# cgisky1980/Qwen3-TTS-Rust

Measured on AMD Instinct MI355X. Metric: audio_sec_per_s, higher is better.
Workload: dtype bf16

## Files before the change

### qwen3-tts-rust_amd/csrc/q3_bgemm.hip

```cpp
#include "q3_kernels.h"

typedef __bf16 bf16x8 __attribute__((ext_vector_type(8)));
typedef uint32_t u32x4 __attribute__((ext_vector_type(4)));

__device__ __forceinline__ float bg_wave_sum(float v) {
#pragma unroll
    for (int m = 32; m >= 1; m >>= 1) v = v + __shfl_xor(v, m);
    return v;
}

__device__ __forceinline__ size_t bg_yoff(const Q3BGemm& g, int row) {
    return g.seg_rows ? (size_t)(row / g.seg_rows) * g.seg_stride + (size_t)(row % g.seg_rows) * g.ldy : (size_t)row * g.ldy;
}
__device__ __forceinline__ float bg_gelu_erf(float x) { return 0.5f * x * (1.0f + erff(x * 0.70710678118654752f)); }

__device__ __forceinline__ u32x4 bg_ldw(const u32x4* p, bool nt) { return nt ? __builtin_nontemporal_load(p) : *p; }

__device__ __forceinline__ bf16x8 bg_q8_frag(uint32_t lo, uint32_t hi) {
    union { u32x4 u; bf16x8 v; } r;
#define Q8F(w_, b_) __float_as_uint((float)(int)(signed char)((w_) >> (8 * (b_))))
    r.u.x = (Q8F(lo, 0) >> 16) | (Q8F(lo, 1) & 0xffff0000u); r.u.y = (Q8F(lo, 2) >> 16) | (Q8F(lo, 3) & 0xffff0000u);
    r.u.z = (Q8F(hi, 0) >> 16) | (Q8F(hi, 1) & 0xffff0000u); r.u.w = (Q8F(hi, 2) >> 16) | (Q8F(hi, 3) & 0xffff0000u);
#undef Q8F
    return r.v;
}
__device__ __forceinline__ float bg_f16(uint32_t bits) { return (float)__builtin_bit_cast(_Float16, (unsigned short)bits); }

#define BG_PH(RT_, NT_) ((8 * (RT_) * (NT_) > 64 && ((RT_) * (NT_)) % 2 == 0) ? 2 : 1)
template <int RT, int NT, int D, bool NTW, bool Q8>
__global__ __launch_bounds__(512) void k_bgemm(Q3BGemm g) {
    extern __shared__ float part[];
    __shared__ float srow[64];
    Q3_STAMP(g, 0);
    constexpr int TR = RT * NT * 4;
    const int wave = threadIdx.x >> 6, lane = threadIdx.x & 63, kq = lane >> 4, r = lane & 15;
    int cg = blockIdx.x, rc = blockIdx.y;
    if (gridDim.y > 1 && (gridDim.x & 7) == 0) {
        const int id = blockIdx.x + gridDim.x * blockIdx.y, G = gridDim.y;
        rc = (id >> 3) % G; cg = (id & 7) + (id / (8 * G)) * 8;
    }
    const int nb0 = cg * NT, row0 = rc * RT * 16, kblocks = g.K >> 5, per = g.K >> 8, kb0 = wave * per;
    const int B = g.B;
    const u32x4* ap[RT];
#pragma unroll
    for (int i = 0; i < RT; ++i) {
        const int R = g.a_row0 + min(row0 + 16 * i + r, B - 1);
        ap[i] = (const u32x4*)g.a + ((size_t)(R >> 4) * kblocks + kb0) * 64 + kq * 16 + (R & 15);
    }
    const u32x4* wp[NT];
#pragma unroll
    for (int j = 0; j < NT; ++j) wp[j] = (const u32x4*)g.w + ((size_t)(nb0 + j) * kblocks + kb0) * 64 + lane;
    constexpr int NR = 2 * RT;
    float sp0[NR], sp1[NR];
    if (g.ssp) {
#pragma unroll
        for (int i = 0; i < NR; ++i) {
            const float* sp = g.ssp + (size_t)min(row0 + wave + 8 * i, B - 1) * g.ld_ssp;
            sp0[i] = lane < g.ntiles ? sp[lane] : 0.0f;
            sp1[i] = lane + 64 < g.ntiles ? sp[lane + 64] : 0.0f;
        }
    }
    constexpr int DQ = (D + 1) & ~1, DP = DQ / 2;
    u32x4 aq[Q8 ? DQ : D][RT], bq[Q8 ? DP : D][NT];
    uint32_t sc8[Q8 ? DP : 1][NT];
    const u32x4* wq[NT]; const uint32_t* sq[NT];
    const int npair = per >> 1;
    if constexpr (Q8) {
#pragma unroll
        for (int j = 0; j < NT; ++j) {
            wq[j] = (const u32x4*)g.w + ((size_t)(nb0 + j) * (kblocks >> 1) + (kb0 >> 1)) * 64 + lane;
            sq[j] = (const uint32_t*)(g.wscale + (size_t)((nb0 + j) * 16 + r) * kblocks + kb0);
        }
#pragma unroll
        for (int p = 0; p < DP; ++p) {
            const int pc = min(p, npair - 1);
#pragma unroll
            for (int j = 0; j < NT; ++j) { bq[p][j] = bg_ldw(wq[j] + (size_t)pc * 64, NTW); sc8[p][j] = sq[j][pc]; }
        }
#pragma unroll
        for (int s = 0; s < DQ; ++s) {
            const size_t so = (size_t)min(s, per - 1) * 64;
#pragma unroll
            for (int i = 0; i < RT; ++i) aq[s][i] = ap[i][so];
        }
    } else {
#pragma unroll
        for (int s = 0; s < D; ++s) {
            const size_t so = (size_t)min(s, per - 1) * 64;
#pragma unroll
            for (int j = 0; j < NT; ++j) bq[s][j] = bg_ldw(wp[j] + so, NTW);
        }
#pragma unroll
        for (int s = 0; s < D; ++s) {
            const size_t so = (size_t)min(s, per - 1) * 64;
#pragma unroll
            for (int i = 0; i < RT; ++i) aq[s][i] = ap[i][so];
        }
    }
    constexpr int NOUT = (TR * 64 + 511) / 512;
    float yres[NOUT], nwv[NOUT], bsv[NOUT], csv[NOUT];
#pragma unroll
    for (int it = 0; it < NOUT; ++it) { yres[it] = 0.0f; nwv[it] = 0.0f; bsv[it] = 0.0f; csv[it] = 1.0f; }
    if (g.epi == Q3_EPI_RESID) {
#pragma unroll
        for (int it = 0; it < NOUT; ++it) {
            const int o = threadIdx.x + it * 512;
            const int l = o & 63, e = (o >> 6) & 3, t = o >> 8, i = t / NT, j = t - i * NT;
            const int row = row0 + 16 * i + 4 * (l >> 4) + e, col = (nb0 + min(j, NT - 1)) * 16 + (l & 15);
            const bool in = o < TR * 64;
            yres[it] = (in && row < B) ? g.y[bg_yoff(g, row) + col] : 0.0f;
            if (g.nw_next) nwv[it] = in ? g.nw_next[col] : 0.0f;
            if (g.col_scale) csv[it] = in ? g.col_scale[col] : 1.0f;
        }
    }
    if (g.bias && g.epi != Q3_EPI_SWIGLU) {
#pragma unroll
        for (int it = 0; it < NOUT; ++it) {
            const int o = threadIdx.x + it * 512;
            const int l = o & 63, t = o >> 8, i = t / NT, j = t - i * NT;
            const int col = (nb0 + min(j, NT - 1)) * 16 + (l & 15);
            bsv[it] = o < TR * 64 ? g.bias[col % g.bias_n] : 0.0f;
        }
    }
    __builtin_amdgcn_sched_barrier(0);
    Q3_STAMP(g, 1);
    if (g.ssp) {
        float av[NR];
#pragma unroll
        for (int i = 0; i < NR; ++i) {
            float a = sp0[i];
            if (lane + 64 < g.ntiles) a = a + sp1[i];
            if (g.ntiles > 128) {
                const float* sp = g.ssp + (size_t)min(row0 + wave + 8 * i, B - 1) * g.ld_ssp;
                for (int t = lane + 128; t < g.ntiles; t += 64) a = a + sp[t];
            }
            av[i] = a;
        }
#pragma unroll
        for (int m = 32; m >= 1; m >>= 1)
#pragma unroll
            for (int i = 0; i < NR; ++i) av[i] = av[i] + __shfl_xor(av[i], m);
        if (lane == 0) {
#pragma unroll
            for (int i = 0; i < NR; ++i) srow[wave + 8 * i] = 1.0f / sqrtf(av[i] / (float)g.d_norm + g.eps);
        }
    }
    __builtin_amdgcn_sched_barrier(0);
    f32x4 acc[RT][NT];
#pragma unroll
    for (int i = 0; i < RT; ++i)
#pragma unroll
        for (int j = 0; j < NT; ++j) acc[i][j] = (f32x4){0.f, 0.f, 0.f, 0.f};
    if constexpr (Q8) {
        const f32x4 zero4 = (f32x4){0.f, 0.f, 0.f, 0.f};
        for (int p0 = 0; p0 < npair; p0 += DP) {
#pragma unroll
            for (int dp = 0; dp < DP; ++dp) {
                const int p = p0 + dp;
                if (p < npair) {
#pragma unroll
                    for (int h = 0; h < 2; ++h) {
                        float dsc[NT]; bf16x8 bf[NT];
#pragma unroll
                        for (int j = 0; j < NT; ++j) {
                            dsc[j] = bg_f16(h ? sc8[dp][j] >> 16 : sc8[dp][j] & 0xffffu);
                            bf[j] = h ? bg_q8_frag(bq[dp][j].z, bq[dp][j].w) : bg_q8_frag(bq[dp][j].x, bq[dp][j].y);
                        }
#pragma unroll
                        for (int i = 0; i < RT; ++i) {
                            union { u32x4 u; bf16x8 v; } a; a.u = aq[2 * dp + h][i];
#pragma unroll
                            for (int j = 0; j < NT; ++j) {
                                const f32x4 P = __builtin_amdgcn_mfma_f32_16x16x32_bf16(a.v, bf[j], zero4, 0, 0, 0);
                                acc[i][j][0] = fmaf(dsc[j], P[0], acc[i][j][0]); acc[i][j][1] = fmaf(dsc[j], P[1], acc[i][j][1]);
                                acc[i][j][2] = fmaf(dsc[j], P[2], acc[i][j][2]); acc[i][j][3] = fmaf(dsc[j], P[3], acc[i][j][3]);
                            }
                        }
                    }
                    __builtin_amdgcn_sched_barrier(0);
                    if (p + DP < npair) {
#pragma unroll
                        for (int j = 0; j < NT; ++j) { bq[dp][j] = bg_ldw(wq[j] + (size_t)(p + DP) * 64, NTW); sc8[dp][j] = sq[j][p + DP]; }
#pragma unroll
                        for (int h = 0; h < 2; ++h)
#pragma unroll
                            for (int i = 0; i < RT; ++i) aq[2 * dp + h][i] = ap[i][(size_t)(2 * (p + DP) + h) * 64];
                    }
                    __builtin_amdgcn_sched_barrier(0);
                }
            }
        }
    } else
    for (int s0 = 0; s0 < per; s0 += D) {
#pragma unroll
        for (int d = 0; d < D; ++d) {
            const int s = s0 + d;
            if (s < per) {
#pragma unroll
                for (int i = 0; i < RT; ++i) {
                    union { u32x4 u; bf16x8 v; } a; a.u = aq[d][i];
#pragma unroll
                    for (int j = 0; j < NT; ++j) {
                        union { u32x4 u; bf16x8 v; } b; b.u = bq[d][j];
                        acc[i][j] = __builtin_amdgcn_mfma_f32_16x16x32_bf16(a.v, b.v, acc[i][j], 0, 0, 0);
                    }
                }
                __builtin_amdgcn_sched_barrier(0);
#ifdef Q3_STAMPS
                if (s == 0) { asm volatile("" :: "v"(acc[0][0][0])); Q3_STAMP(g, 2); }
#endif
                if (s + D < per) {
#pragma unroll
                    for (int j = 0; j < NT; ++j) bq[d][j] = bg_ldw(wp[j] + (size_t)(s + D) * 64, NTW);
#pragma unroll
                    for (int i = 0; i < RT; ++i) aq[d][i] = ap[i][(size_t)(s + D) * 64];
                }
                __builtin_amdgcn_sched_barrier(0);
            }
        }
    }
#ifdef Q3_STAMPS
    asm volatile("" :: "v"(acc[0][0][0])); Q3_STAMP(g, 3);
#endif
    constexpr int PH = BG_PH(RT, NT), TP = RT * NT / PH, TRP = TR / PH, NOUTP = NOUT / PH;
    static_assert(PH == 1 || ((RT * NT) % 2 == 0 && (TRP * 64) % 512 == 0), "two phases need an even tile count and whole items per phase");
    const int epi = g.epi;
#pragma unroll
    for (int ph = 0; ph < PH; ++ph) {
        if (ph) __syncthreads();
#pragma unroll
        for (int i = 0; i < RT; ++i)
#pragma unroll
            for (int j = 0; j < NT; ++j) {
                if ((i * NT + j) / TP != ph) continue;
#pragma unroll
                for (int e = 0; e < 4; ++e) part[((size_t)wave * TRP + ((i * NT + j) - ph * TP) * 4 + e) * 64 + lane] = acc[i][j][e];
            }
        __syncthreads();
        if (ph == 0) Q3_STAMP(g, 4);
        if (epi == Q3_EPI_SWIGLU) {
            constexpr int NP = (TRP * 32 + 511) / 512;
#pragma unroll
            for (int it = 0; it < NP; ++it) {
                const int p = threadIdx.x + it * 512;
                if (p >= TRP * 32) break;
                const int q = p & 31, l = ((q >> 3) << 4) + (q & 7), o = ((p >> 5) << 6) + l;
                const int e = (o >> 6) & 3, t = ph * TP + (o >> 8), i = t / NT, j = t - i * NT;
                const int rl = 16 * i + 4 * (l >> 4) + e, row = row0 + rl, c = l & 15;
                const float sc = g.ssp ? srow[rl] : 1.0f;
                float gt = part[o], up = part[o + 8];
#pragma unroll
                for (int wv = 1; wv < 8; ++wv) { gt = gt + part[(size_t)wv * (TRP * 64) + o]; up = up + part[(size_t)wv * (TRP * 64) + o + 8]; }
                if (row < B) g.yb[q3_atile_off(row, (nb0 + j) * 8 + c, g.N >> 6)] = q3_bf16(q3_swiglu(sc * gt, sc * up));
            }
            continue;
        }
#pragma unroll
        for (int itp = 0; itp < NOUTP; ++itp) {
            const int it = ph * NOUTP + itp, o = threadIdx.x + itp * 512;
            if (o >= TRP * 64) break;
            const int l = o & 63, e = (o >> 6) & 3, t = ph * TP + (o >> 8), i = t / NT, j = t - i * NT;
            const int rl = 16 * i + 4 * (l >> 4) + e, row = row0 + rl, c = l & 15;
            const int col = (nb0 + j) * 16 + c;
            const bool live = row < B;
            const float sc = g.ssp ? srow[rl] : 1.0f;
            float v = part[o];
#pragma unroll
            for (int wv = 1; wv < 8; ++wv) v = v + part[(size_t)wv * (TRP * 64) + o];
            if (g.bias) v = v + bsv[it];
            if (epi == Q3_EPI_STORE) {
                if (live) g.y[bg_yoff(g, row) + col] = g.ssp ? sc * v : v;
            } else if (epi == Q3_EPI_GELU) {
                if (live) g.yb[q3_atile_off(row, col, g.N >> 5)] = q3_bf16(bg_gelu_erf(v));
            } else if (epi == Q3_EPI_RESID) {
                const float xv = g.col_scale ? yres[it] + csv[it] * v : yres[it] + v;
                if (live) g.y[bg_yoff(g, row) + col] = xv;
                if (g.yb && !g.nw_next && live) g.yb[q3_atile_off(row, col, g.N >> 5)] = q3_bf16(xv);
                if (g.nw_next) {
                    if (live) g.yb[q3_atile_off(row, col, g.N >> 5)] = q3_bf16(xv * nwv[it]);
                    float sq = xv * xv;
                    sq = sq + __shfl_xor(sq, 1); sq = sq + __shfl_xor(sq, 2); sq = sq + __shfl_xor(sq, 4); sq = sq + __shfl_xor(sq, 8);
                    if (live && c == 0) g.ssp_out[(size_t)row * g.ld_ssp_out + (nb0 + j)] = sq;
                }
            } else {
                unsigned long long key = q3_argmax_key(g.ssp ? sc * v : v, (uint32_t)col);
#pragma unroll
                for (int m = 1; m <= 8; m <<= 1) { const unsigned long long ok = __shfl_xor(key, m); key = ok > key ? ok : key; }
                if (live && c == 0) g.keys[(size_t)row * g.key_stride + (nb0 + j)] = key;
            }
        }
    }
#ifdef Q3_STAMPS
    Q3_STAMP(g, 5);
    asm volatile("s_waitcnt vmcnt(0)" ::: "memory");
    Q3_STAMP(g, 6);
#endif
}

#define BB_NS 4
__global__ __launch_bounds__(256) void k_bgemm_big(Q3BGemm g) {
    extern __shared__ __attribute__((aligned(16))) char bb_ring[];
    __shared__ float srow[128];
    const int tid = threadIdx.x, wave = tid >> 6, lane = tid & 63, wm = wave >> 1, wn = wave & 1, kq = lane >> 4, c = lane & 15;
    int bx = blockIdx.x, by = blockIdx.y;
    {
        const int total = gridDim.x * gridDim.y;
        if ((total & 7) == 0) {
            const int id = blockIdx.x + gridDim.x * blockIdx.y, t = (id & 7) * (total >> 3) + (id >> 3);
            by = t % gridDim.y; bx = t / gridDim.y;
        }
    }
    const int B = g.B, kblocks = g.K >> 5, per = g.K >> 8;
    const int rt0 = (g.a_row0 >> 4) + by * 8, rt_last = (g.a_row0 + B - 1) >> 4, nb0 = bx * 8;
    const u32x4* asrc[2]; const u32x4* bsrc[2];
#pragma unroll
    for (int i = 0; i < 2; ++i) {
        asrc[i] = (const u32x4*)g.a + (size_t)min(rt0 + wave * 2 + i, rt_last) * kblocks * 64 + lane;
        bsrc[i] = (const u32x4*)g.w + (size_t)(nb0 + wave * 2 + i) * kblocks * 64 + lane;
    }
    auto issue = [&](int step) {
        char* st = bb_ring + (size_t)(step % BB_NS) * 16384;
#pragma unroll
        for (int i = 0; i < 2; ++i) {
            __builtin_amdgcn_global_load_lds((const __attribute__((address_space(1))) void*)(asrc[i] + (size_t)step * 64),
                                             (__attribute__((address_space(3))) void*)(st + (wave * 2 + i) * 1024), 16, 0, 0);
            __builtin_amdgcn_global_load_lds((const __attribute__((address_space(1))) void*)(bsrc[i] + (size_t)step * 64),
                                             (__attribute__((address_space(3))) void*)(st + 8192 + (wave * 2 + i) * 1024), 16, 0, 0);
        }
    };
#pragma unroll
    for (int p = 0; p < BB_NS - 1; ++p) issue(p);
    if (g.ssp) {
        for (int i0 = 0; i0 < 32; i0 += 16) {
            float a0[16], a1[16];
#pragma unroll
            for (int i = 0; i < 16; ++i) {
                const float* sp = g.ssp + (size_t)min(by * 128 + wave + 4 * (i0 + i), B - 1) * g.ld_ssp;
                a0[i] = lane < g.ntiles ? sp[lane] : 0.0f;
                a1[i] = lane + 64 < g.ntiles ? sp[lane + 64] : 0.0f;
            }
#pragma unroll
            for (int i = 0; i < 16; ++i) {
                float a = a0[i];
                if (lane + 64 < g.ntiles) a = a + a1[i];
                if (g.ntiles > 128) {
                    const float* sp = g.ssp + (size_t)min(by * 128 + wave + 4 * (i0 + i), B - 1) * g.ld_ssp;
                    for (int t = lane + 128; t < g.ntiles; t += 64) a = a + sp[t];
                }
                a0[i] = a;
            }
#pragma unroll
            for (int m = 32; m >= 1; m >>= 1)
#pragma unroll
                for (int i = 0; i < 16; ++i) a0[i] = a0[i] + __shfl_xor(a0[i], m);
            if (lane == 0) {
#pragma unroll
                for (int i = 0; i < 16; ++i) srow[wave + 4 * (i0 + i)] = 1.0f / sqrtf(a0[i] / (float)g.d_norm + g.eps);
            }
        }
    }
    f32x4 acc[4][4], tot[4][4];
    const int nsteps = kblocks;
    int in_slice = 0, slice = 0;
#pragma unroll
    for (int i = 0; i < 4; ++i)
#pragma unroll
        for (int j = 0; j < 4; ++j) acc[i][j] = (f32x4){0.f, 0.f, 0.f, 0.f};
    for (int step = 0; step < nsteps; ++step) {
        if (step + BB_NS - 2 < nsteps) asm volatile("s_waitcnt vmcnt(%0)" ::"n"((BB_NS - 2) * 4) : "memory");
        else asm volatile("s_waitcnt vmcnt(0)" ::: "memory");
        Q3_LDS_BARRIER();
        if (step + BB_NS - 1 < nsteps) issue(step + BB_NS - 1);
        const char* st = bb_ring + (size_t)(step % BB_NS) * 16384;
        bf16x8 a_[4], b_[4];
#pragma unroll
        for (int i = 0; i < 4; ++i) a_[i] = *(const bf16x8*)(st + (wm * 4 + i) * 1024 + lane * 16);
#pragma unroll
        for (int j = 0; j < 4; ++j) b_[j] = *(const bf16x8*)(st + 8192 + (wn * 4 + j) * 1024 + lane * 16);
#pragma unroll
        for (int i = 0; i < 4; ++i)
#pragma unroll
            for (int j = 0; j < 4; ++j) acc[i][j] = __builtin_amdgcn_mfma_f32_16x16x32_bf16(a_[i], b_[j], acc[i][j], 0, 0, 0);
        if (++in_slice == per) {
#pragma unroll
            for (int i = 0; i < 4; ++i)
#pragma unroll
                for (int j = 0; j < 4; ++j) {
                    if (slice == 0) tot[i][j] = acc[i][j];
                    else { tot[i][j][0] = tot[i][j][0] + acc[i][j][0]; tot[i][j][1] = tot[i][j][1] + acc[i][j][1]; tot[i][j][2] = tot[i][j][2] + acc[i][j][2]; tot[i][j][3] = tot[i][j][3] + acc[i][j][3]; }
                    acc[i][j] = (f32x4){0.f, 0.f, 0.f, 0.f};
                }
            in_slice = 0; ++slice;
        }
    }
    __syncthreads();
    const int epi = g.epi;
    if (epi == Q3_EPI_RESID) {
#pragma unroll
        for (int i = 0; i < 4; ++i)
#pragma unroll
            for (int j = 0; j < 4; ++j)
#pragma unroll
                for (int e = 0; e < 4; ++e) {
                    const int row = min(by * 128 + wm * 64 + i * 16 + 4 * kq + e, B - 1);
                    acc[i][j][e] = g.y[(size_t)row * g.ldy + (nb0 + wn * 4 + j) * 16 + c];
                }
    }
#pragma unroll
    for (int i = 0; i < 4; ++i)
#pragma unroll
        for (int e = 0; e < 4; ++e) {
            const int rl = wm * 64 + i * 16 + 4 * kq + e, row = by * 128 + rl;
            const bool live = row < B;
            const float sc = g.ssp ? srow[rl] : 1.0f;
#pragma unroll
            for (int j = 0; j < 4; ++j) {
                const int tile = nb0 + wn * 4 + j, col = tile * 16 + c;
                const float v = tot[i][j][e];
                if (epi == Q3_EPI_SWIGLU) {
                    const float up = __shfl(v, (lane + 8) & 63);
                    if (live && c < 8) g.yb[q3_atile_off(row, tile * 8 + c, g.N >> 6)] = q3_bf16(q3_swiglu(sc * v, sc * up));
                } else if (epi == Q3_EPI_STORE) {
                    if (live) g.y[(size_t)row * g.ldy + col] = g.ssp ? sc * v : v;
                } else {
                    const float xv = acc[i][j][e] + v;
                    if (live) g.y[(size_t)row * g.ldy + col] = xv;
                    if (g.nw_next) {
                        if (live) g.yb[q3_atile_off(row, col, g.N >> 5)] = q3_bf16(xv * g.nw_next[col]);
                        float sq = xv * xv;
                        sq = sq + __shfl_xor(sq, 1); sq = sq + __shfl_xor(sq, 2); sq = sq + __shfl_xor(sq, 4); sq = sq + __shfl_xor(sq, 8);
                        if (live && c == 0) g.ssp_out[(size_t)row * g.ld_ssp_out + tile] = sq;
                    }
                }
            }
        }
}
static bool bg_big_ok(const Q3BGemm& g) {
    return g.B >= 256 && !g.wscale && (g.epi == Q3_EPI_STORE || g.epi == Q3_EPI_RESID || g.epi == Q3_EPI_SWIGLU) && g.N % 128 == 0 && g.a_row0 % 16 == 0 &&
           !g.bias && !g.col_scale && !g.seg_rows && !(g.epi == Q3_EPI_RESID && g.yb && !g.nw_next);
}
static void bg_launch_big(const Q3BGemm& g, hipStream_t s) {
    const dim3 grid(g.N / 128, (g.B + 127) / 128);
    hipLaunchKernelGGL(k_bgemm_big, grid, dim3(256), BB_NS * 16384, s, g);
}

template <int RT, int NT>
struct BgInst {
    static constexpr int S = RT + NT;
    static constexpr int D = S <= 3 ? 8 : (S == 4 ? 5 : (S == 5 ? 4 : (S == 6 ? 3 : 2)));
    static constexpr size_t lds = (size_t)8 * RT * NT * 4 * 64 * 4 / BG_PH(RT, NT);
    static void prepare() {
        if (lds > 65536) {
            hipFuncSetAttribute((const void*)k_bgemm<RT, NT, D, false, false>, hipFuncAttributeMaxDynamicSharedMemorySize, (int)lds);
            hipFuncSetAttribute((const void*)k_bgemm<RT, NT, D, true, false>, hipFuncAttributeMaxDynamicSharedMemorySize, (int)lds);
            hipFuncSetAttribute((const void*)k_bgemm<RT, NT, D, false, true>, hipFuncAttributeMaxDynamicSharedMemorySize, (int)lds);
            hipFuncSetAttribute((const void*)k_bgemm<RT, NT, D, true, true>, hipFuncAttributeMaxDynamicSharedMemorySize, (int)lds);
        }
    }
    static void launch(const Q3BGemm& g, dim3 grid, hipStream_t s) {
        const bool nt = g.w_once && grid.y == 1;
        if (g.wscale) {
            if (nt) hipLaunchKernelGGL((k_bgemm<RT, NT, D, true, true>), grid, dim3(512), lds, s, g);
            else hipLaunchKernelGGL((k_bgemm<RT, NT, D, false, true>), grid, dim3(512), lds, s, g);
        } else if (nt) hipLaunchKernelGGL((k_bgemm<RT, NT, D, true, false>), grid, dim3(512), lds, s, g);
        else hipLaunchKernelGGL((k_bgemm<RT, NT, D, false, false>), grid, dim3(512), lds, s, g);
    }
};
#define BG_EACH(X) X(1, 1) X(1, 2) X(1, 3) X(2, 1) X(2, 2) X(2, 3) X(3, 1) X(3, 2) X(3, 3) X(4, 1) X(4, 2) X(4, 3)
static int g_lds_cap_kb = 0;
static int g_big_policy = 0;
void q3_bgemm_prepare() {
    static Q3PerDevice pd;
    static std::once_flag env_once;
    std::call_once(env_once, []() {
        const char* ev = getenv("Q3TTS_BG_BIG"); g_big_policy = ev ? atoi(ev) : 0;
        ev = getenv("Q3TTS_BG_LDS_CAP"); g_lds_cap_kb = ev ? atoi(ev) : 0;
    });
    pd.ensure(1, []() {
        hipFuncSetAttribute((const void*)k_bgemm_big, hipFuncAttributeMaxDynamicSharedMemorySize, BB_NS * 16384);
#define P(RT_, NT_) BgInst<RT_, NT_>::prepare();
        BG_EACH(P)
#undef P
    });
}

static int g_force_rt = 0, g_force_nt = 0;
void q3_bgemm_force(int rt, int nt) { g_force_rt = rt; g_force_nt = nt; }
void q3_bgemm_big_policy(int policy) { q3_bgemm_prepare(); g_big_policy = policy; }

static void bg_pick(const Q3BGemm& g, int* rt, int* nt, int* big) {
    *big = 0;
    if (g.B >= 256 && g_force_rt == 0 && bg_big_ok(g)) {
        const int policy = g_big_policy;
        const long wgs = (long)(g.N / 128) * ((g.B + 127) / 128);
        if (policy > 0 || (policy == 0 && wgs >= 256)) { *big = 1; *rt = 8; *nt = 8; return; }
    }
    const int tiles = g.N / 16;
    int bestRT = 1, bestNT = 1; long bestCost = -1, bestWgs = 0;
    for (int RT = 1; RT <= 4; ++RT)
        for (int NT = 1; NT <= 3; ++NT) {
            if (tiles % NT) continue;
            if (g_lds_cap_kb > 0 && 8 * RT * NT / BG_PH(RT, NT) > g_lds_cap_kb && !(RT == 1 && NT == 1)) continue;
            if (g.B > 64 && RT != 4 && !(RT == 2 && g.B <= 128)) continue;
            const long chunks = (g.B + 16 * RT - 1) / (16 * RT);
            if (g.B <= 64 && RT > 1 && 16 * (RT - 1) * chunks >= g.B) continue;
            const long wgs = (long)(tiles / NT) * chunks, rounds = (wgs + 255) / 256;
            const long cost = rounds * ((g.wscale ? 32L * RT + 17L * NT : 32L * (RT + NT)) * g.K + 24000L);
            if (bestCost < 0 || cost < bestCost || (cost == bestCost && (wgs > bestWgs || (wgs == bestWgs && NT > bestNT)))) { bestCost = cost; bestRT = RT; bestNT = NT; bestWgs = wgs; }
        }
    if (g_force_rt > 0 && g_force_nt > 0 && tiles % g_force_nt == 0) { bestRT = g_force_rt; bestNT = g_force_nt; }
    *rt = bestRT; *nt = bestNT;
}
void q3_bgemm_pick(const Q3BGemm& g, int* rt, int* nt, int* d, int* ntw, int* big) {
    q3_bgemm_prepare();
    bg_pick(g, rt, nt, big);
    *d = 0; *ntw = 0;
    if (*big) return;
#define X(RT_, NT_) if (*rt == RT_ && *nt == NT_) *d = BgInst<RT_, NT_>::D;
    BG_EACH(X)
#undef X
    *ntw = (g.w_once && (g.B + 16 * *rt - 1) / (16 * *rt) == 1) ? 1 : 0;
}

static int bg_check(const Q3BGemm& g) {
    if (g.B < 1 || g.N % 16 || g.K % 256 || g.K < 256 || !g.a || !g.w || g.a_row0 < 0) return -1;
    if (g.wscale && g.K % 512) return -1;
    if (g.yb && (((g.epi == Q3_EPI_RESID || g.epi == Q3_EPI_GELU) && g.N % 32) || (g.epi == Q3_EPI_SWIGLU && g.N % 64))) return -1;
    if ((g.epi == Q3_EPI_SWIGLU || g.epi == Q3_EPI_GELU) && (!g.yb)) return -1;
    if (g.bias && g.bias_n < 1) return -1;
    if (g.ssp && g.ntiles < 1) return -1;
    return 0;
}

int q3_launch_bgemm(const Q3BGemm& g, hipStream_t s) {
    if (bg_check(g)) return -1;
    q3_bgemm_prepare();
    int bestRT, bestNT, big;
    bg_pick(g, &bestRT, &bestNT, &big);
    if (big) { bg_launch_big(g, s); return 0; }
    const dim3 grid(g.N / 16 / bestNT, (g.B + 16 * bestRT - 1) / (16 * bestRT));
#define L(RT_, NT_) if (bestRT == RT_ && bestNT == NT_) { BgInst<RT_, NT_>::launch(g, grid, s); return 0; }
    BG_EACH(L)
#undef L
    return -1;
}

__global__ __launch_bounds__(256) void k_norm_inputs(const float* x, int ldx, int d, const float* nw, uint16_t* xb, int xb_row0, float* ssp, int ld_ssp) {
    const int row = blockIdx.x;
    for (int i = threadIdx.x; i < d; i += 256)
        q3_norm_out(x[(size_t)row * ldx + i], nw[i], xb + q3_atile_off(xb_row0 + row, i, d >> 5), ssp + (size_t)row * ld_ssp + (i >> 4), (i & 15) == 0);
}
__global__ __launch_bounds__(256) void k_norm_inputs_q8(const float* x, int ldx, int d, const float* nw, int8_t* xq, uint16_t* xscale, int rt16, float* ssp, int ld_ssp) {
    const int row = blockIdx.x;
    for (int i = threadIdx.x; i < d; i += 256) {
        const float v = x[(size_t)row * ldx + i];
        q3_q8_out32(v * nw[i], row, i, d >> 6, rt16, xq, xscale);
        float sq = v * v;
        sq = sq + __shfl_xor(sq, 1); sq = sq + __shfl_xor(sq, 2); sq = sq + __shfl_xor(sq, 4); sq = sq + __shfl_xor(sq, 8);
        if ((i & 15) == 0) ssp[(size_t)row * ld_ssp + (i >> 4)] = sq;
    }
}
void q3_launch_norm_inputs_q8(const float* x, int ldx, int rows, int d, const float* nw, int8_t* xq, uint16_t* xscale, int rt16, float* ssp, int ld_ssp, hipStream_t s) {
    hipLaunchKernelGGL(k_norm_inputs_q8, dim3(rows), dim3(256), 0, s, x, ldx, d, nw, xq, xscale, rt16, ssp, ld_ssp);
}
void q3_launch_norm_inputs(const float* x, int ldx, int rows, int d, const float* nw, uint16_t* xb, int xb_row0, float* ssp, int ld_ssp, hipStream_t s) {
    hipLaunchKernelGGL(k_norm_inputs, dim3(rows), dim3(256), 0, s, x, ldx, d, nw, xb, xb_row0, ssp, ld_ssp);
}
```

### qwen3-tts-rust_amd/csrc/q3_engine.h

```cpp
#pragma once
#include <algorithm>
#include <atomic>
#include <mutex>
#include <string>
#include <vector>

#include "../../include/q3tts.h"
#include "q3_kernels.h"

struct Q3Voc;
struct Q3Mel;
struct Q3Clone;

struct Q3Tfm {
    int L = 0, d = 0, Hq = 0, Hkv = 0, hd = 0, F = 0, nq = 0, nkv = 0, nqkv = 0, head_n = 0;
    std::vector<float*> attn_norm, ffn_norm, qn, kn;
    std::vector<uint4*> wqkv, wo, wgu, wd;
    float* out_norm = nullptr;
    uint4* head = nullptr;
    std::vector<uint16_t*> sqkv, so, sgu, sd; uint16_t* shead = nullptr; bool q8 = false;
    bool a8 = false;
    uint16_t *kc = nullptr, *vc = nullptr;
    size_t layer_stride = 0;
    int n_ctx = 0, n_slots = 0;
    float *cs = nullptr, *sn = nullptr;
    size_t weight_bytes = 0;
};

struct Q3Scratch {
    float* qkv = nullptr;
    uint16_t *att = nullptr, *h = nullptr;
    uint16_t *asc_att = nullptr, *asc_h = nullptr; int rt16 = 0;
    int rows = 0;
};

struct Q3Lane {
    int nb = 0;
    hipStream_t stream = nullptr;
    float *xT = nullptr, *logits = nullptr, *logits_tmp = nullptr, *fb = nullptr, *px = nullptr;
    uint16_t *xbT = nullptr, *xbP = nullptr;
    float *sspT = nullptr, *sspP = nullptr;
    uint16_t* ascT = nullptr; int rt16T = 0;
    unsigned long long* keys = nullptr;
    int *row_pos_t = nullptr, *slot_id = nullptr, *posA = nullptr, *slotA = nullptr, *pos_q = nullptr, *perm = nullptr;
    Q3Scratch sc;
    std::vector<hipGraph_t> graphs;
    std::vector<hipGraphExec_t> execs;
    hipEvent_t ev_begin = nullptr, ev_end = nullptr;
};

struct q3tts_engine {
    q3tts_engine_config cfg;
    std::string err;
    hipStream_t stream = nullptr, vstream = nullptr;
    Q3Tfm T, P;
    float* text = nullptr;
    std::vector<float*> codec;
    const float** codec_dev = nullptr;
    std::vector<float*> pproj;
    float* proj_w = nullptr;
    float* proj_b = nullptr;
    float* tts_pad = nullptr;
    float* tts_pad_own = nullptr;
    float* marker_row = nullptr;
    int B = 0;
    std::vector<int> buckets; int cur_bucket = -1;
    std::vector<int> row_of_slot, slot_of_row;
    Q3Slot* slots = nullptr;
    Q3Slot* slots_host = nullptr;
    int* codes = nullptr;
    float* rng = nullptr;
    std::vector<Q3Lane> lanes;
    Q3Scratch sc_pre;
    float* xp = nullptr;
    uint16_t* xbp = nullptr; float* sspp = nullptr;
    uint16_t* ascp = nullptr; int rt16p = 0;
    int *pf_pos = nullptr, *pf_slot = nullptr;
    int* pf_seg = nullptr;
    Q3PromptRow* prow_dev = nullptr; int prow_cap = 0;
    float* spk_dev = nullptr; int* refcodes_dev = nullptr;
    float temperature = 0.7f; int top_k = 40; float top_p = 0.9f; int has_seed = 0; uint64_t seed = 0;
    int max_steps = 512;
    hipEvent_t ev0 = nullptr, ev1 = nullptr, ev2 = nullptr, ev3 = nullptr;
    std::vector<hipEvent_t> fin_ev;
    q3tts_timings tm{};
    Q3Voc* voc = nullptr;
    Q3Mel* mel = nullptr;
    Q3Clone* clone = nullptr;
    int probe = 0, probe_kind = 0;
    std::vector<hipEvent_t> probe_ev;
    int probe_i = 0;
    double probe_ms = 0, probe_empty_ms = 0; long long probe_cnt = 0, probe_empty_cnt = 0, row_steps = 0;
    int dev_pcm_on = 0; float* dev_pcm = nullptr; int dev_pcm_n = 0; size_t dev_pcm_stride = 0;
    double hp_launch = 0, hp_sync = 0;
    float* first_chunk_host = nullptr;
    std::atomic<q3tts_session*> session{nullptr};
    std::mutex err_mu;
};

int q3_set_err(q3tts_engine* e, int code, const std::string& msg);
int q3_refuse_in_session(q3tts_engine* e);
#define Q3_NOT_IN_SESSION(e) do { if ((e) && (e)->session.load()) return q3_refuse_in_session(e); } while (0)
#define Q3_HIP(e, call)                                                                                         \
    do {                                                                                                        \
        hipError_t err__ = (call);                                                                              \
        if (err__ != hipSuccess)                                                                                \
            return q3_set_err((e), Q3TTS_ERR_DEVICE, std::string(#call) + ": " + hipGetErrorString(err__));     \
    } while (0)

int q3_dev_alloc_zeroed(q3tts_engine* e, void** p, size_t bytes);

void q3_stdrng_f32(uint64_t seed, int n, float* out);

void q3_mel_destroy(q3tts_engine* e);
int q3_mel_run(q3tts_engine* e, const float* audio, int64_t n_samples, int32_t* n_frames, float** out_dev);
void q3_clone_destroy(q3tts_engine* e);
int q3_voc_create(q3tts_engine* e);
void q3_voc_destroy(q3tts_engine* e);
int q3_voc_reset(q3tts_engine* e, int slot);
int q3_voc_decode(q3tts_engine* e, int slot, int f0, int nf, int is_last, hipStream_t s);
int q3_voc_decode_batch(q3tts_engine* e, const int* slots, const int* real, int ns, int nf, hipStream_t s, int beside_decoder);
void q3_voc_mark_last(q3tts_engine* e, int slot);
float* q3_voc_pcm(q3tts_engine* e, int slot);
int q3_voc_samples(q3tts_engine* e, int slot);
int q3_voc_samples_per_frame(const q3tts_engine* e);
size_t q3_voc_pcm_stride(const q3tts_engine* e);

int q3_plan_rows(q3tts_engine* e, const std::vector<int>& live);
int q3_admit_many(q3tts_engine* e, const int* slots, const q3tts_request* const* reqs, int count, int* rc);
int q3_run_chunk(q3tts_engine* e, int CH);
int q3_voc_dispatch(q3tts_engine* e, const char* live, const char* want, int* voc_frames, bool more, bool* first);
double q3_now_ms();
```

### qwen3-tts-rust_amd/csrc/q3_engine.hip

```cpp
#include "q3_engine.h"
#include "q3_gguf.h"

#include <chrono>
#include <cmath>
#include <cstdio>
#include <cstdlib>
#include <cstring>

static thread_local std::string g_err;

int q3_set_err(q3tts_engine* e, int code, const std::string& msg) {
    if (e) { std::lock_guard<std::mutex> lk(e->err_mu); e->err = msg; }
    g_err = msg;
    return code;
}
extern "C" const char* q3tts_last_error(const q3tts_engine* e) {
    if (!e) return g_err.c_str();
    if (!e->session.load()) return e->err.c_str();
    static thread_local std::string copy;
    std::lock_guard<std::mutex> lk(const_cast<q3tts_engine*>(e)->err_mu);
    copy = e->err;
    return copy.c_str();
}
int q3_refuse_in_session(q3tts_engine* e) {
    return q3_set_err(e, Q3TTS_ERR_STATE, "the engine is owned by an open session (q3tts_session_close first)");
}

extern "C" void q3tts_default_config(q3tts_engine_config* c) {
    memset(c, 0, sizeof(*c));
    q3tts_model_config& m = c->model;
    m.t_n_layer = 28; m.t_d_model = 2048; m.t_n_head = 16; m.t_n_kv_head = 8; m.t_head_dim = 128; m.t_d_ffn = 6144;
    m.t_vocab = 3072; m.t_rope_theta = 1000000.0f;
    m.t_mrope_sections[0] = 24; m.t_mrope_sections[1] = 20; m.t_mrope_sections[2] = 20; m.t_mrope_sections[3] = 0;
    m.p_n_layer = 5; m.p_d_model = 1024; m.p_n_head = 16; m.p_n_kv_head = 8; m.p_head_dim = 128; m.p_d_ffn = 3072;
    m.p_rope_theta = 1000000.0f;
    m.n_codebooks = 16; m.codebook_size = 2048; m.rms_eps = 1e-6f;
    m.d_embed = 2048; m.text_vocab = 151936; m.codec0_rows = 3072; m.codecq_rows = 2048;
    m.sample_limit = 2160; m.eos_code = 2150; m.tts_pad_id = 151671;
    q3tts_vocoder_config& v = c->vocoder;
    v.n_codebooks = 16; v.codebook_size = 2048; v.codebook_dim = 512; v.latent_dim = 1024; v.pre_conv_kernel = 3;
    v.n_layer = 8; v.n_head = 16; v.head_dim = 64; v.d_ffn = 3072; v.sliding_window = 72;
    v.rope_theta = 10000.0f; v.rms_eps = 1e-5f; v.layer_scale_init = 0.01f;
    v.n_upsample = 2; v.upsample_ratios[0] = 2; v.upsample_ratios[1] = 2;
    v.decoder_dim = 1536; v.n_dec_blocks = 4;
    v.dec_rates[0] = 8; v.dec_rates[1] = 5; v.dec_rates[2] = 4; v.dec_rates[3] = 3;
    v.lookahead_frames = 0; v.sample_rate = 24000;
    c->device = 0; c->max_batch = 1; c->n_ctx = 4096; c->max_steps_cap = 512; c->with_vocoder = 1;
    c->synth_seed = 0; c->weights_path = nullptr; c->talker_q8_0 = 0; c->vocoder_flush_tail = 0;
}

static int validate(const q3tts_engine_config& c, std::string& why) {
    const q3tts_model_config& m = c.model;
#define REQ(cond) do { if (!(cond)) { why = "config check failed: " #cond; return Q3TTS_ERR_INVALID; } } while (0)
    REQ(m.t_n_layer > 0 && m.p_n_layer > 0);
    REQ(m.t_head_dim == 128 && m.p_head_dim == 128);
    REQ(m.t_d_model % 512 == 0 && m.p_d_model % 512 == 0 && m.t_d_ffn % 512 == 0 && m.p_d_ffn % 512 == 0);
    REQ(m.t_d_model <= 8192 && m.p_d_model <= 8192);
    REQ((m.t_n_head * m.t_head_dim) % 512 == 0 && (m.p_n_head * m.p_head_dim) % 512 == 0);
    REQ(m.t_n_head % m.t_n_kv_head == 0 && m.p_n_head % m.p_n_kv_head == 0);
    { int r = m.t_n_head / m.t_n_kv_head; REQ(r == 1 || r == 2 || r == 4); r = m.p_n_head / m.p_n_kv_head; REQ(r == 1 || r == 2 || r == 4); }
    REQ(m.t_vocab % 16 == 0 && m.codebook_size % 16 == 0 && m.t_d_ffn % 8 == 0);
    REQ(m.d_embed == m.t_d_model);
    REQ(m.d_embed % 512 == 0);
    REQ(m.n_codebooks >= 2 && m.n_codebooks <= 16);
    REQ(m.sample_limit > 0 && m.sample_limit <= m.t_vocab && m.sample_limit <= 4096);
    REQ(m.t_mrope_sections[0] + m.t_mrope_sections[1] + m.t_mrope_sections[2] + m.t_mrope_sections[3] == m.t_head_dim / 2);
    REQ(m.tts_pad_id >= 0 && m.tts_pad_id < m.text_vocab);
    REQ(c.max_batch >= 1 && c.max_batch <= 64);
    REQ(c.n_ctx >= 64 && c.n_ctx % 64 == 0 && c.n_ctx <= 8192);
    REQ(c.max_steps_cap >= 1 && c.max_steps_cap < c.n_ctx);
    REQ(m.n_codebooks + 1 <= 64);
    REQ(c.talker_q8_0 >= 0 && c.talker_q8_0 <= 2);
    if (c.talker_q8_0) REQ(m.t_d_model % 512 == 0 && m.t_d_ffn % 512 == 0 && (m.t_n_head * m.t_head_dim) % 512 == 0);
    if (c.talker_q8_0 == 2) REQ(m.t_vocab % 32 == 0 && ((m.t_n_head + 2 * m.t_n_kv_head) * m.t_head_dim) % 32 == 0 && m.t_d_ffn % 64 == 0);
#undef REQ
    return Q3TTS_OK;
}

int q3_dev_alloc_zeroed(q3tts_engine* e, void** p, size_t bytes) {
    void* q = nullptr;
    hipError_t err = hipMalloc(&q, bytes);
    if (err != hipSuccess) return q3_set_err(e, Q3TTS_ERR_OOM, std::string("hipMalloc: ") + hipGetErrorString(err));
    err = hipMemsetAsync(q, 0, bytes, e->stream);
    if (err == hipSuccess) err = hipStreamSynchronize(e->stream);
    if (err != hipSuccess) { hipFree(q); return q3_set_err(e, Q3TTS_ERR_DEVICE, std::string("hipMemset: ") + hipGetErrorString(err)); }
    *p = q;
    return Q3TTS_OK;
}
template <class T>
static int dalloc(q3tts_engine* e, T** p, size_t n) {
    void* q = nullptr;
    const int rc = q3_dev_alloc_zeroed(e, &q, n * sizeof(T) + 64);
    if (rc != Q3TTS_OK) return rc;
    *p = (T*)q;
    return Q3TTS_OK;
}
#define TRY(x) do { int rc__ = (x); if (rc__ != Q3TTS_OK) return rc__; } while (0)

static void rope_tables(int n_pos, int hd, float theta, const int* sections, std::vector<float>& cs, std::vector<float>& sn) {
    const int half = hd / 2;
    int s3 = half;
    if (sections) s3 = sections[0] + sections[1] + sections[2];
    cs.resize((size_t)n_pos * half); sn.resize((size_t)n_pos * half);
    for (int p = 0; p < n_pos; ++p)
        for (int i = 0; i < half; ++i) {
            const double inv = pow((double)theta, -2.0 * (double)i / (double)hd);
            const double ang = (i < s3) ? (double)p * inv : 0.0;
            cs[(size_t)p * half + i] = (float)cos(ang);
            sn[(size_t)p * half + i] = (float)sin(ang);
        }
}

struct GgSrc {
    q3tts_engine* e; const Q3Gguf* g; const char* file;
    std::vector<uint16_t> host; uint16_t* dev[2] = {nullptr, nullptr}; size_t dev_cap[2] = {0, 0};
    ~GgSrc() { for (auto p : dev) if (p) hipFree(p); for (auto p : dev8) if (p) hipFree(p); }
    int fail(const std::string& msg) { return q3_set_err(e, Q3TTS_ERR_INVALID, std::string(file) + ": " + msg); }
    const Q3GgufTensor* need(const std::string& name, uint64_t ne0, uint64_t ne1, int* rc) {
        const Q3GgufTensor* t = g->find(name);
        if (!t) { *rc = fail("tensor '" + name + "' is missing"); return nullptr; }
        const uint64_t d1 = t->dims.size() > 1 ? t->dims[1] : 1;
        if (t->dims[0] != ne0 || d1 != ne1 || t->dims.size() > 2) {
            *rc = fail("tensor '" + name + "' has shape [" + std::to_string(d1) + "][" + std::to_string(t->dims[0]) + "], the configuration needs [" +
                       std::to_string(ne1) + "][" + std::to_string(ne0) + "]");
            return nullptr;
        }
        *rc = Q3TTS_OK;
        return t;
    }
    int vec(const std::string& name, size_t n, float* dst) {
        int rc; const Q3GgufTensor* t = need(name, n, 1, &rc);
        if (!t) return rc;
        std::vector<float> h(n); std::string err;
        if (q3_gguf_to_f32(*t, h.data(), err)) return fail(err);
        Q3_HIP(e, hipMemcpy(dst, h.data(), n * 4, hipMemcpyHostToDevice));
        return Q3TTS_OK;
    }
    uint8_t* dev8[2] = {nullptr, nullptr}; size_t dev8_cap[2] = {0, 0}; bool raw[2] = {false, false};
    int mat_q8(const std::string& name, size_t N, size_t K, int which) {
        int rc; const Q3GgufTensor* t = need(name, K, N, &rc);
        if (!t) return rc;
        raw[which] = false;
        if (t->type != Q3_GGML_Q8_0) return mat(name, N, K, which);
        const size_t bytes = N * (K / 32) * 34;
        if (t->nbytes < bytes) return fail("tensor '" + name + "' is shorter than its Q8_0 shape");
        if (dev8_cap[which] < bytes) {
            if (dev8[which]) hipFree(dev8[which]);
            dev8[which] = nullptr; dev8_cap[which] = 0;
            void* p = nullptr;
            if (hipMalloc(&p, bytes) != hipSuccess) return q3_set_err(e, Q3TTS_ERR_OOM, "hipMalloc (Q8_0 staging)");
            dev8[which] = (uint8_t*)p; dev8_cap[which] = bytes;
        }
        Q3_HIP(e, hipMemcpy(dev8[which], t->data, bytes, hipMemcpyHostToDevice));
        raw[which] = true;
        return Q3TTS_OK;
    }
    int mat(const std::string& name, size_t N, size_t K, int which) {
        int rc; const Q3GgufTensor* t = need(name, K, N, &rc);
        if (!t) return rc;
        host.resize(N * K); std::string err;
        if (q3_gguf_to_bf16(*t, host.data(), err)) return fail(err);
        if (dev_cap[which] < N * K) {
            if (dev[which]) hipFree(dev[which]);
            dev[which] = nullptr; dev_cap[which] = 0;
            void* p = nullptr;
            if (hipMalloc(&p, N * K * 2) != hipSuccess) return q3_set_err(e, Q3TTS_ERR_OOM, "hipMalloc (weight staging)");
            dev[which] = (uint16_t*)p; dev_cap[which] = N * K;
        }
        Q3_HIP(e, hipMemcpy(dev[which], host.data(), N * K * 2, hipMemcpyHostToDevice));
        return Q3TTS_OK;
    }
};

static int init_tfm(q3tts_engine* e, Q3Tfm& t, int grp, int L, int d, int Hq, int Hkv, int hd, int F, int head_n, float theta,
                    const int* sections, int n_ctx, int n_slots, GgSrc* gg = nullptr, int q8mode = 0) {
    const bool q8 = q8mode != 0;
    t.L = L; t.d = d; t.Hq = Hq; t.Hkv = Hkv; t.hd = hd; t.F = F; t.nq = Hq * hd; t.nkv = Hkv * hd; t.nqkv = t.nq + 2 * t.nkv;
    t.head_n = head_n; t.n_ctx = n_ctx; t.n_slots = n_slots; t.q8 = q8; t.a8 = q8mode == 2;
    const uint64_t seed = e->cfg.synth_seed;
    const float ms = 0.02f / Q3_IH4_STD, ns = 0.05f / Q3_IH4_STD;
    hipStream_t s = e->stream;
    t.attn_norm.resize(L); t.ffn_norm.resize(L); t.qn.resize(L); t.kn.resize(L);
    t.wqkv.resize(L); t.wo.resize(L); t.wgu.resize(L); t.wd.resize(L);
    if (q8) { t.sqkv.assign(L, nullptr); t.so.assign(L, nullptr); t.sgu.assign(L, nullptr); t.sd.assign(L, nullptr); }
    const size_t wdiv = q8 ? 16 : 8;
    auto alloc_mat = [&](uint4** w, uint16_t** sc, size_t N, size_t K) -> int {
        TRY(dalloc(e, w, N * K / wdiv));
        if (q8) TRY(dalloc(e, sc, N * K / 32));
        return Q3TTS_OK;
    };
    auto fill = [&](Q3Fill& f, uint16_t* sc) { if (q8) { f.dst_scale = sc; q3_launch_fill_tiled_q8(f, s); } else q3_launch_fill_tiled(f, s); };
    const double bpw = q8 ? 1.0625 : 2.0;
    for (int l = 0; l < L; ++l) {
        TRY(dalloc(e, &t.attn_norm[l], (size_t)d)); TRY(dalloc(e, &t.ffn_norm[l], (size_t)d));
        TRY(dalloc(e, &t.qn[l], (size_t)hd)); TRY(dalloc(e, &t.kn[l], (size_t)hd));
        uint16_t *sc_qkv = nullptr, *sc_o = nullptr, *sc_gu = nullptr, *sc_d = nullptr;
        TRY(alloc_mat(&t.wqkv[l], &sc_qkv, t.nqkv, d)); TRY(alloc_mat(&t.wo[l], &sc_o, d, t.nq));
        TRY(alloc_mat(&t.wgu[l], &sc_gu, (size_t)2 * F, d)); TRY(alloc_mat(&t.wd[l], &sc_d, d, F));
        if (q8) { t.sqkv[l] = sc_qkv; t.so[l] = sc_o; t.sgu[l] = sc_gu; t.sd[l] = sc_d; }
        t.weight_bytes += (size_t)(bpw * (double)((size_t)t.nqkv * d + (size_t)d * t.nq + 3ull * F * d));
        if (gg) {
            const std::string b = "blk." + std::to_string(l) + ".";
            Q3_HIP(e, hipStreamSynchronize(s));
            TRY(gg->vec(b + "attn_norm.weight", d, t.attn_norm[l])); TRY(gg->vec(b + "ffn_norm.weight", d, t.ffn_norm[l]));
            TRY(gg->vec(b + "attn_q_norm.weight", hd, t.qn[l])); TRY(gg->vec(b + "attn_k_norm.weight", hd, t.kn[l]));
            Q3Fill f{}; f.mode = 0;
            auto stage = [&](const std::string& name, size_t N, size_t K, int which) -> int { return q8 ? gg->mat_q8(name, N, K, which) : gg->mat(name, N, K, which); };
            auto put = [&](const std::string& name, uint4* dst, uint16_t* sc, int Ntot, int K, int row0, int rows) -> int {
                TRY(stage(name, rows, K, 0));
                f.dst = dst; f.N = Ntot; f.K = K; f.mode = 0; f.row0 = row0; f.rows = rows; f.src_b = nullptr; f.src8_b = nullptr;
                f.src_a = (q8 && gg->raw[0]) ? nullptr : gg->dev[0]; f.src8_a = (q8 && gg->raw[0]) ? gg->dev8[0] : nullptr;
                fill(f, sc);
                Q3_HIP(e, hipStreamSynchronize(s));
                return Q3TTS_OK;
            };
            TRY(put(b + "attn_q.weight", t.wqkv[l], sc_qkv, t.nqkv, d, 0, t.nq));
            TRY(put(b + "attn_k.weight", t.wqkv[l], sc_qkv, t.nqkv, d, t.nq, t.nkv));
            TRY(put(b + "attn_v.weight", t.wqkv[l], sc_qkv, t.nqkv, d, t.nq + t.nkv, t.nkv));
            TRY(put(b + "attn_output.weight", t.wo[l], sc_o, d, t.nq, 0, d));
            TRY(stage(b + "ffn_gate.weight", F, d, 0)); TRY(stage(b + "ffn_up.weight", F, d, 1));
            f.dst = t.wgu[l]; f.N = 2 * F; f.K = d; f.mode = 1;
            f.src_a = (q8 && gg->raw[0]) ? nullptr : gg->dev[0]; f.src8_a = (q8 && gg->raw[0]) ? gg->dev8[0] : nullptr;
            f.src_b = (q8 && gg->raw[1]) ? nullptr : gg->dev[1]; f.src8_b = (q8 && gg->raw[1]) ? gg->dev8[1] : nullptr;
            if (q8 && gg->raw[0] != gg->raw[1]) return gg->fail("ffn_gate / ffn_up of block " + std::to_string(l) + " differ in type (one Q8_0, one not)");
            fill(f, sc_gu);
            Q3_HIP(e, hipStreamSynchronize(s));
            TRY(put(b + "ffn_down.weight", t.wd[l], sc_d, d, F, 0, d));
            continue;
        }
        q3_launch_fill_f32(t.attn_norm[l], d, seed, Q3_TID(grp, l, Q3W_ATTN_NORM), 1.0f, ns, 0, s);
        q3_launch_fill_f32(t.ffn_norm[l], d, seed, Q3_TID(grp, l, Q3W_FFN_NORM), 1.0f, ns, 0, s);
        q3_launch_fill_f32(t.qn[l], hd, seed, Q3_TID(grp, l, Q3W_QNORM), 1.0f, ns, 0, s);
        q3_launch_fill_f32(t.kn[l], hd, seed, Q3_TID(grp, l, Q3W_KNORM), 1.0f, ns, 0, s);
        Q3Fill f{}; f.seed = seed; f.scale = ms;
        f.dst = t.wqkv[l]; f.N = t.nqkv; f.K = d; f.mode = 0;
        f.row0 = 0; f.rows = t.nq; f.tid_a = Q3_TID(grp, l, Q3W_Q); fill(f, sc_qkv);
        f.row0 = t.nq; f.rows = t.nkv; f.tid_a = Q3_TID(grp, l, Q3W_K); fill(f, sc_qkv);
        f.row0 = t.nq + t.nkv; f.rows = t.nkv; f.tid_a = Q3_TID(grp, l, Q3W_V); fill(f, sc_qkv);
        f.dst = t.wo[l]; f.N = d; f.K = t.nq; f.row0 = 0; f.rows = d; f.tid_a = Q3_TID(grp, l, Q3W_O); fill(f, sc_o);
        f.dst = t.wgu[l]; f.N = 2 * F; f.K = d; f.mode = 1; f.tid_a = Q3_TID(grp, l, Q3W_GATE); f.tid_b = Q3_TID(grp, l, Q3W_UP);
        fill(f, sc_gu);
        f.dst = t.wd[l]; f.N = d; f.K = F; f.mode = 0; f.row0 = 0; f.rows = d; f.tid_a = Q3_TID(grp, l, Q3W_DOWN); fill(f, sc_d);
    }
    TRY(dalloc(e, &t.out_norm, (size_t)d));
    TRY(alloc_mat(&t.head, &t.shead, (size_t)head_n, d));
    t.weight_bytes += (size_t)(bpw * (double)((size_t)head_n * d));
    if (gg) {
        Q3_HIP(e, hipStreamSynchronize(s));
        TRY(gg->vec("output_norm.weight", d, t.out_norm));
        TRY(q8 ? gg->mat_q8("output.weight", head_n, d, 0) : gg->mat("output.weight", head_n, d, 0));
        Q3Fill f{}; f.dst = t.head; f.N = head_n; f.K = d; f.mode = 0; f.row0 = 0; f.rows = head_n;
        f.src_a = (q8 && gg->raw[0]) ? nullptr : gg->dev[0]; f.src8_a = (q8 && gg->raw[0]) ? gg->dev8[0] : nullptr;
        fill(f, t.shead);
        Q3_HIP(e, hipStreamSynchronize(s));
    } else {
        q3_launch_fill_f32(t.out_norm, d, seed, Q3_TID(grp, Q3_L_MODEL, Q3WM_OUT_NORM), 1.0f, ns, 0, s);
        Q3Fill f{}; f.seed = seed; f.scale = ms; f.dst = t.head; f.N = head_n; f.K = d; f.mode = 0; f.row0 = 0; f.rows = head_n;
        f.tid_a = Q3_TID(grp, Q3_L_MODEL, Q3WM_HEAD); fill(f, t.shead);
    }
    t.layer_stride = (size_t)n_slots * Hkv * n_ctx * hd;
    TRY(dalloc(e, &t.kc, t.layer_stride * L)); TRY(dalloc(e, &t.vc, t.layer_stride * L));
    std::vector<float> cs, sn;
    rope_tables(n_ctx, hd, theta, sections, cs, sn);
    TRY(dalloc(e, &t.cs, cs.size())); TRY(dalloc(e, &t.sn, sn.size()));
    Q3_HIP(e, hipMemcpyAsync(t.cs, cs.data(), cs.size() * 4, hipMemcpyHostToDevice, s));
    Q3_HIP(e, hipMemcpyAsync(t.sn, sn.data(), sn.size() * 4, hipMemcpyHostToDevice, s));
    Q3_HIP(e, hipStreamSynchronize(s));
    return Q3TTS_OK;
}
static void free_tfm(Q3Tfm& t) {
    for (auto p : t.attn_norm) hipFree(p); for (auto p : t.ffn_norm) hipFree(p); for (auto p : t.qn) hipFree(p);
    for (auto p : t.kn) hipFree(p); for (auto p : t.wqkv) hipFree(p); for (auto p : t.wo) hipFree(p);
    for (auto p : t.wgu) hipFree(p); for (auto p : t.wd) hipFree(p);
    hipFree(t.out_norm); hipFree(t.head); hipFree(t.kc); hipFree(t.vc); hipFree(t.cs); hipFree(t.sn);
    for (auto p : t.sqkv) hipFree(p); for (auto p : t.so) hipFree(p); for (auto p : t.sgu) hipFree(p); for (auto p : t.sd) hipFree(p);
    hipFree(t.shead);
}

static int alloc_scratch(q3tts_engine* e, Q3Scratch& sc, int rows, int nqkv, int nq, int F, int dmax) {
    sc.rows = rows;
    const size_t r16 = ((size_t)rows + 15) & ~(size_t)15;
    TRY(dalloc(e, &sc.qkv, (size_t)rows * nqkv)); TRY(dalloc(e, &sc.att, r16 * nq)); TRY(dalloc(e, &sc.h, r16 * F));
    sc.rt16 = (int)(r16 / 16);
    if (e->T.a8) { TRY(dalloc(e, &sc.asc_att, r16 * (nq / 32))); TRY(dalloc(e, &sc.asc_h, r16 * (F / 32))); }
    return Q3TTS_OK;
}

static int run_layers(q3tts_engine* e, Q3Tfm& t, float* x, uint16_t* xb, float* ssp, int rows, const int* row_pos, const int* row_slot, Q3Scratch& sc,
                       hipStream_t s, bool one_row_per_slot = false, hipEvent_t* probe = nullptr, int slot_mod = 0, int pos_const = 0,
                       const int* seg = nullptr, int n_seg = 0, int seg_max_n = 0, uint16_t* xscale = nullptr, int x_rt16 = 0) {
    auto gemm = [&](Q3BGemm& g) { return t.a8 ? q3_launch_bgemm8(g, s) : q3_launch_bgemm(g, s); };
    const float eps = e->cfg.model.rms_eps;
    int bad = 0;
    const int nt = t.d / 16;
    const int once = &t == &e->T ? 1 : 0;
    for (int l = 0; l < t.L; ++l) {
        Q3BGemm g{};
        g.w_once = once;
        g.a = xb; g.B = rows; g.w = t.wqkv[l]; g.wscale = t.q8 ? t.sqkv[l] : nullptr; g.K = t.d; g.N = t.nqkv; g.ssp = ssp; g.ld_ssp = nt; g.ntiles = nt; g.d_norm = t.d; g.eps = eps;
        g.epi = Q3_EPI_STORE; g.y = sc.qkv; g.ldy = t.nqkv;
        if (t.a8) { g.ascale = xscale; g.a_rt16 = x_rt16; }
        const int pk = (probe && l == 0) ? e->probe_kind : -1;
        if (pk == 1) hipEventRecord(probe[0], s);
        bad += gemm(g) != 0;
        if (pk == 1) hipEventRecord(probe[1], s);
        Q3QkPrep qp{}; qp.qkv = sc.qkv; qp.ld = t.nqkv; qp.rows = rows; qp.Hq = t.Hq; qp.Hkv = t.Hkv; qp.hd = t.hd;
        qp.qnw = t.qn[l]; qp.knw = t.kn[l]; qp.eps = eps; qp.cs = t.cs; qp.sn = t.sn;
        qp.kc = t.kc + l * t.layer_stride; qp.vc = t.vc + l * t.layer_stride; qp.n_ctx = t.n_ctx; qp.row_pos = row_pos; qp.row_slot = row_slot;
        qp.slot_mod = slot_mod; qp.pos_const = pos_const;
        const bool fused = one_row_per_slot && t.Hq / t.Hkv >= 2;
        const bool pair = !one_row_per_slot && slot_mod > 0 && rows == 2 * slot_mod && pos_const == 0 && t.Hq / t.Hkv == 2 && t.hd == 128;
        if (!fused && !pair) q3_launch_qk_prep(qp, s);
        Q3Attend at{}; at.qkv = sc.qkv; at.ld = t.nqkv; at.rows = rows; at.out = (float*)sc.att; at.ldo = t.nq; at.Hq = t.Hq; at.Hkv = t.Hkv; at.hd = t.hd;
        at.kc = qp.kc; at.vc = qp.vc; at.n_ctx = t.n_ctx; at.row_pos = row_pos; at.row_slot = row_slot;
        at.fused = pair ? 2 : (fused ? 1 : 0); at.prep = qp; at.out_bf16 = 1; at.slot_mod = slot_mod; at.pos_const = pos_const;
        if (t.a8) { at.out_bf16 = 2; at.out_scale = sc.asc_att; at.out_rt16 = sc.rt16; }
        if (!fused && !pair && n_seg > 0) { at.seg = seg; at.n_seg = n_seg; at.seg_max_n = seg_max_n; }
        if (pk == 2) hipEventRecord(probe[0], s);
        q3_launch_attend(at, s);
        if (pk == 2) hipEventRecord(probe[1], s);
        g = Q3BGemm{}; g.w_once = once; g.a = sc.att; g.B = rows; g.w = t.wo[l]; g.wscale = t.q8 ? t.so[l] : nullptr; g.K = t.nq; g.N = t.d; g.epi = Q3_EPI_RESID; g.y = x; g.ldy = t.d;
        g.yb = xb; g.nw_next = t.ffn_norm[l]; g.ssp_out = ssp; g.ld_ssp_out = nt;
        if (t.a8) { g.ascale = sc.asc_att; g.a_rt16 = sc.rt16; g.yscale = xscale; g.y_rt16 = x_rt16; }
        if (pk == 3) hipEventRecord(probe[0], s);
        bad += gemm(g) != 0;
        if (pk == 3) hipEventRecord(probe[1], s);
        g = Q3BGemm{}; g.w_once = once; g.a = xb; g.B = rows; g.w = t.wgu[l]; g.wscale = t.q8 ? t.sgu[l] : nullptr; g.K = t.d; g.N = 2 * t.F; g.ssp = ssp; g.ld_ssp = nt; g.ntiles = nt; g.d_norm = t.d;
        g.eps = eps; g.epi = Q3_EPI_SWIGLU; g.yb = sc.h;
        if (t.a8) { g.ascale = xscale; g.a_rt16 = x_rt16; g.yscale = sc.asc_h; g.y_rt16 = sc.rt16; }
        if (pk == 0) hipEventRecord(probe[0], s);
        bad += gemm(g) != 0;
        if (pk == 0) hipEventRecord(probe[1], s);
        g = Q3BGemm{}; g.w_once = once; g.a = sc.h; g.B = rows; g.w = t.wd[l]; g.wscale = t.q8 ? t.sd[l] : nullptr; g.K = t.F; g.N = t.d; g.epi = Q3_EPI_RESID; g.y = x; g.ldy = t.d;
        g.yb = xb; g.nw_next = l + 1 < t.L ? t.attn_norm[l + 1] : t.out_norm; g.ssp_out = ssp; g.ld_ssp_out = nt;
        if (t.a8) { g.ascale = sc.asc_h; g.a_rt16 = sc.rt16; g.yscale = xscale; g.y_rt16 = x_rt16; }
        if (pk == 4) hipEventRecord(probe[0], s);
        bad += gemm(g) != 0;
        if (pk == 4) hipEventRecord(probe[1], s);
    }
    return bad;
}

static int record_frame(q3tts_engine* e, Q3Lane& L, hipStream_t s, int B) {
    int bad = 0;
    const q3tts_model_config& m = e->cfg.model;
    const int ncb = m.n_codebooks, cbs = m.codebook_size, dp = m.p_d_model, de = m.d_embed, cap = e->cfg.max_steps_cap;
    const float eps = m.rms_eps;
    Q3Slot* slots = e->slots;
    int* codes = e->codes;
    Q3Sample sa{}; sa.logits = L.logits; sa.ld = m.t_vocab; sa.limit = m.sample_limit; sa.eos = m.eos_code; sa.slots = slots; sa.B = B; sa.row_slot = L.slot_id;
    sa.rng = e->rng; sa.codes = codes; sa.max_steps_cap = cap; sa.ncb = ncb;
    Q3PredInput pi{}; pi.xT = L.xT; pi.out_norm = e->T.out_norm; pi.eps = eps; pi.d = de; pi.codec0 = e->codec[0]; pi.codec0_rows = m.codec0_rows;
    pi.slots = slots; pi.row_slot = L.slot_id; pi.X = nullptr; pi.fb = L.fb; pi.B = B; pi.pproj0 = e->pproj[0]; pi.proj_b = e->proj_b; pi.dp = dp; pi.px = L.px;
    pi.nw = e->P.attn_norm[0]; pi.xb = L.xbP; pi.ssp = L.sspP;
    {
        Q3Project pj{}; pj.x = L.xT; pj.ldx = de; pj.rows = B; pj.w = e->proj_w; pj.bias = e->proj_b; pj.n_in = de; pj.n_out = dp; pj.y = L.px; pj.ldy = dp;
        pj.nw = e->P.attn_norm[0]; pj.xb = L.xbP; pj.ssp = L.sspP; pj.ld_ssp = dp / 16;
        pj.norm_w = e->T.out_norm; pj.eps = eps;
        bad += q3_launch_sample_input(sa, pi, pj, s) != 0;
    }
    const size_t head_tile_stride = (size_t)(cbs / 16) * (dp / 32) * 64;
    auto pred_next = [&](int q) {
        Q3PredNext pn{}; pn.keys = L.keys; pn.n_key_parts = cbs / 16; pn.q = q; pn.ncb = ncb; pn.codec_q = e->codec[q]; pn.rows_q = m.codecq_rows; pn.d = de;
        pn.slots = slots; pn.row_slot = L.slot_id; pn.B = B; pn.codes = codes; pn.max_steps_cap = cap; pn.fb = L.fb;
        pn.tts_pad = e->tts_pad; pn.xT = L.xT; pn.row_pos_t = L.row_pos_t; pn.pproj_q = e->pproj[q]; pn.proj_b = e->proj_b; pn.dp = dp; pn.px = L.px;
        const bool last = q == ncb - 1;
        pn.nw = last ? e->T.attn_norm[0] : e->P.attn_norm[0]; pn.xb = last ? L.xbT : L.xbP; pn.ssp = last ? L.sspT : L.sspP;
        if (last && e->T.a8) { pn.xscale = L.ascT; pn.x_rt16 = L.rt16T; }
        q3_launch_pred_next(pn, s);
    };
    for (int q = 0; q < ncb - 1; ++q) {
        const int rows = q == 0 ? 2 * B : B;
        if (q > 0) pred_next(q);
        hipEvent_t* pe = nullptr;
        if (e->probe == 1 && q == 1 && B == L.nb && e->probe_i + 2 <= 8) { pe = &e->probe_ev[e->probe_i]; e->probe_i += 2; }
        bad += run_layers(e, e->P, L.px, L.xbP, L.sspP, rows, nullptr, nullptr, L.sc, s, q > 0, pe, B, q == 0 ? 0 : q + 1);
        Q3BGemm g{}; g.a = L.xbP; g.a_row0 = q == 0 ? B : 0; g.B = B; g.w = e->P.head + head_tile_stride * q; g.K = dp; g.N = cbs;
        g.ssp = q == 0 ? L.sspP + (size_t)B * (dp / 16) : L.sspP; g.ld_ssp = dp / 16; g.ntiles = dp / 16; g.d_norm = dp; g.eps = eps;
        g.epi = Q3_EPI_ARGMAX; g.keys = L.keys; g.key_stride = cbs / 16;
        bad += q3_launch_bgemm(g, s) != 0;
    }
    pred_next(ncb - 1);
    hipEvent_t* pt = nullptr;
    if (e->probe == 2 && B == L.nb && e->probe_i + 2 <= 8) { pt = &e->probe_ev[e->probe_i]; e->probe_i += 2; }
    bad += run_layers(e, e->T, L.xT, L.xbT, L.sspT, B, L.row_pos_t, L.slot_id, L.sc, s, true, pt, 0, 0, nullptr, 0, 0, L.ascT, L.rt16T);
    Q3BGemm g{}; g.w_once = 1; g.a = L.xbT; g.B = B; g.w = e->T.head; g.wscale = e->T.q8 ? e->T.shead : nullptr; g.K = m.t_d_model; g.N = m.t_vocab;
    g.ssp = L.sspT; g.ld_ssp = m.t_d_model / 16; g.ntiles = m.t_d_model / 16; g.d_norm = m.t_d_model; g.eps = eps;
    g.epi = Q3_EPI_STORE; g.y = L.logits; g.ldy = m.t_vocab;
    if (e->T.a8) { g.ascale = L.ascT; g.a_rt16 = L.rt16T; bad += q3_launch_bgemm8(g, s) != 0; }
    else bad += q3_launch_bgemm(g, s) != 0;
    return bad;
}

static bool file_exists(const std::string& p) { FILE* f = fopen(p.c_str(), "rb"); if (f) fclose(f); return f != nullptr; }
static uint16_t host_bf16(float f) {
    uint32_t u; memcpy(&u, &f, 4);
    if ((u & 0x7fffffffu) > 0x7f800000u) return (uint16_t)((u >> 16) | 0x40u);
    return (uint16_t)((u + 0x7fffu + ((u >> 16) & 1u)) >> 16);
}
static int upload_table(q3tts_engine* e, float** dst, const float* host, size_t n) {
    TRY(dalloc(e, dst, n));
    Q3_HIP(e, hipMemcpy(*dst, host, n * 4, hipMemcpyHostToDevice));
    return Q3TTS_OK;
}
static int upload_proj(q3tts_engine* e, const float* w, const float* b) {
    const q3tts_model_config& m = e->cfg.model;
    TRY(upload_table(e, &e->proj_w, w, (size_t)m.p_d_model * m.d_embed));
    return upload_table(e, &e->proj_b, b, (size_t)m.p_d_model);
}
static int load_assets_files(q3tts_engine* e, const std::string& dir) {
    q3tts_model_config& m = e->cfg.model;
    const size_t d = (size_t)m.d_embed;
    std::vector<std::vector<float>> tabs(1 + m.n_codebooks);
    std::vector<size_t> rows(1 + m.n_codebooks, 0);
    std::vector<float> pw, pb;
    std::string err;
    const std::string gpath = dir + "/qwen3_assets.gguf";
    if (file_exists(gpath)) {
        Q3Gguf g;
        if (g.open(gpath, err)) return q3_set_err(e, Q3TTS_ERR_INVALID, err);
        auto fetch = [&](const std::string& name, uint64_t ne0, bool required, std::vector<float>& out, size_t* nrows) -> int {
            const Q3GgufTensor* t = g.find(name);
            if (!t) return required ? q3_set_err(e, Q3TTS_ERR_INVALID, gpath + ": " + name + " (tensor) missing") : Q3TTS_OK;
            if (t->dims[0] != ne0 || t->dims.size() > 2) return q3_set_err(e, Q3TTS_ERR_INVALID, gpath + ": tensor '" + name + "' has the wrong row length");
            out.resize(t->nelem);
            if (q3_gguf_to_f32(*t, out.data(), err)) return q3_set_err(e, Q3TTS_ERR_INVALID, gpath + ": " + err);
            if (nrows) *nrows = t->dims.size() > 1 ? (size_t)t->dims[1] : 1;
            return Q3TTS_OK;
        };
        size_t pr = 0;
        TRY(fetch("proj.weight", d, true, pw, &pr));
        if (pr != (size_t)m.p_d_model) return q3_set_err(e, Q3TTS_ERR_INVALID, gpath + ": proj.weight does not have p_d_model rows");
        TRY(fetch("proj.bias", (uint64_t)m.p_d_model, true, pb, nullptr));
        TRY(fetch("text_embd", d, false, tabs[0], &rows[0]));
        for (int q = 0; q < m.n_codebooks; ++q) TRY(fetch("codec_embd." + std::to_string(q), d, true, tabs[1 + q], &rows[1 + q]));
    } else {
        auto fetch = [&](const std::string& file, bool required, std::vector<float>& out, size_t* nrows, size_t row_len) -> int {
            const std::string path = dir + "/" + file;
            if (!file_exists(path)) return required ? q3_set_err(e, Q3TTS_ERR_INVALID, "neither qwen3_assets.gguf nor " + file + " in " + dir) : Q3TTS_OK;
            std::vector<size_t> shape;
            if (q3_npy_load_f32(path, out, shape, err)) return q3_set_err(e, Q3TTS_ERR_INVALID, err);
            if (out.size() % row_len) return q3_set_err(e, Q3TTS_ERR_INVALID, path + ": size is not a multiple of the row length");
            if (nrows) *nrows = out.size() / row_len;
            return Q3TTS_OK;
        };
        size_t pr = 0, br = 0;
        TRY(fetch("proj_weight.npy", true, pw, &pr, d));
        TRY(fetch("proj_bias.npy", true, pb, &br, 1));
        if (pr != (size_t)m.p_d_model || br != (size_t)m.p_d_model) return q3_set_err(e, Q3TTS_ERR_INVALID, dir + ": projection shape does not match p_d_model");
        TRY(fetch("text_embedding_projected.npy", false, tabs[0], &rows[0], d));
        for (int q = 0; q < m.n_codebooks; ++q) TRY(fetch("codec_embedding_" + std::to_string(q) + ".npy", true, tabs[1 + q], &rows[1 + q], d));
    }
    for (int q = 2; q < m.n_codebooks; ++q)
        if (rows[1 + q] != rows[2]) return q3_set_err(e, Q3TTS_ERR_INVALID, dir + ": codec tables 1.." + std::to_string(m.n_codebooks - 1) + " differ in size");
    m.text_vocab = (int32_t)rows[0]; m.codec0_rows = (int32_t)rows[1];
    if (m.n_codebooks > 1) m.codecq_rows = (int32_t)rows[2];
    if (rows[0]) TRY(upload_table(e, &e->text, tabs[0].data(), tabs[0].size()));
    e->codec.resize(m.n_codebooks);
    for (int q = 0; q < m.n_codebooks; ++q) TRY(upload_table(e, &e->codec[q], tabs[1 + q].data(), tabs[1 + q].size()));
    TRY(upload_proj(e, pw.data(), pb.data()));
    if ((size_t)m.tts_pad_id < rows[0]) e->tts_pad = e->text + (size_t)m.tts_pad_id * d;
    else { TRY(dalloc(e, &e->tts_pad_own, d)); Q3_HIP(e, hipMemset(e->tts_pad_own, 0, d * 4)); e->tts_pad = e->tts_pad_own; }
    return Q3TTS_OK;
}

extern "C" int q3tts_engine_create(const q3tts_engine_config* cfg, q3tts_engine** out) {
    if (!cfg || !out) return q3_set_err(nullptr, Q3TTS_ERR_INVALID, "null argument");
    std::string why;
    if (validate(*cfg, why) != Q3TTS_OK) return q3_set_err(nullptr, Q3TTS_ERR_INVALID, why);
    int ndev = 0;
    if (hipGetDeviceCount(&ndev) != hipSuccess || ndev <= 0)
        return q3_set_err(nullptr, Q3TTS_ERR_DEVICE, "no HIP device: libq3tts has no CPU fallback");
    if (cfg->device < 0 || cfg->device >= ndev) return q3_set_err(nullptr, Q3TTS_ERR_INVALID, "device ordinal out of range");
    q3tts_engine* e = new q3tts_engine();
    e->cfg = *cfg; e->cfg.weights_path = nullptr;
    e->max_steps = cfg->max_steps_cap < 512 ? cfg->max_steps_cap : 512;
    auto fail = [&](int rc) { std::string m = e->err; q3tts_engine_destroy(e); g_err = m; return rc; };
#define TRYC(x) do { int rc__ = (x); if (rc__ != Q3TTS_OK) return fail(rc__); } while (0)
#define HIPC(call) do { hipError_t er__ = (call); if (er__ != hipSuccess) { q3_set_err(e, Q3TTS_ERR_DEVICE, std::string(#call) + ": " + hipGetErrorString(er__)); return fail(Q3TTS_ERR_DEVICE); } } while (0)
    HIPC(hipSetDevice(cfg->device));
    q3_bgemm_prepare();
    HIPC(hipStreamCreateWithFlags(&e->stream, hipStreamNonBlocking));
    if (getenv("Q3TTS_VOC_SERIAL") && atoi(getenv("Q3TTS_VOC_SERIAL"))) e->vstream = e->stream;
    else if (getenv("Q3TTS_VOC_CUMASK")) {
        uint32_t w = (uint32_t)strtoul(getenv("Q3TTS_VOC_CUMASK"), nullptr, 16), mask[8];
        for (auto& x : mask) x = w;
        HIPC(hipExtStreamCreateWithCUMask(&e->vstream, 8, mask));
    } else HIPC(hipStreamCreateWithFlags(&e->vstream, hipStreamNonBlocking));
    HIPC(hipEventCreate(&e->ev0)); HIPC(hipEventCreate(&e->ev1)); HIPC(hipEventCreate(&e->ev2)); HIPC(hipEventCreate(&e->ev3));
    e->fin_ev.resize(cfg->max_batch, nullptr);
    for (auto& ev : e->fin_ev) HIPC(hipEventCreateWithFlags(&ev, hipEventDisableTiming));
    q3tts_model_config& m = e->cfg.model;
    const int B = cfg->max_batch;
    e->B = B;
    hipStream_t s = e->stream;
    const std::string wdir = cfg->weights_path ? cfg->weights_path : "";
    Q3Gguf gt, gp;
    GgSrc st{e, &gt, "qwen3_tts_talker.gguf"}, sp{e, &gp, "qwen3_tts_predictor.gguf"};
    if (!wdir.empty()) {
        std::string er;
        if (gt.open(wdir + "/qwen3_tts_talker.gguf", er) || gp.open(wdir + "/qwen3_tts_predictor.gguf", er)) { q3_set_err(e, Q3TTS_ERR_INVALID, er); return fail(Q3TTS_ERR_INVALID); }
    }
    TRYC(init_tfm(e, e->T, Q3G_TALKER, m.t_n_layer, m.t_d_model, m.t_n_head, m.t_n_kv_head, m.t_head_dim, m.t_d_ffn, m.t_vocab,
                  m.t_rope_theta, m.t_mrope_sections, cfg->n_ctx, B, wdir.empty() ? nullptr : &st, cfg->talker_q8_0));
    TRYC(init_tfm(e, e->P, Q3G_PRED, m.p_n_layer, m.p_d_model, m.p_n_head, m.p_n_kv_head, m.p_head_dim, m.p_d_ffn,
                  (m.n_codebooks - 1) * m.codebook_size, m.p_rope_theta, nullptr, 64, B, wdir.empty() ? nullptr : &sp));
    const uint64_t seed = cfg->synth_seed;
    const float es = 0.05f / Q3_IH4_STD;
    if (!wdir.empty()) {
        TRYC(load_assets_files(e, wdir));
        { void* cd = nullptr; HIPC(hipMalloc(&cd, sizeof(float*) * 16)); e->codec_dev = (const float**)cd; }
        HIPC(hipMemcpyAsync((void*)e->codec_dev, e->codec.data(), sizeof(float*) * m.n_codebooks, hipMemcpyHostToDevice, s));
    } else {
    TRYC(dalloc(e, &e->text, (size_t)m.text_vocab * m.d_embed));
    q3_launch_fill_f32(e->text, (size_t)m.text_vocab * m.d_embed, seed, Q3_TID(Q3G_ASSET, 0, Q3WA_TEXT), 0.0f, es, 1, s);
    e->codec.resize(m.n_codebooks);
    for (int q = 0; q < m.n_codebooks; ++q) {
        const size_t rows = q == 0 ? m.codec0_rows : m.codecq_rows;
        TRYC(dalloc(e, &e->codec[q], rows * m.d_embed));
        q3_launch_fill_f32(e->codec[q], rows * m.d_embed, seed, Q3_TID(Q3G_ASSET, 1 + q, 0), 0.0f, es, 1, s);
    }
    { void* cd = nullptr; HIPC(hipMalloc(&cd, sizeof(float*) * 16)); e->codec_dev = (const float**)cd; }
    HIPC(hipMemcpyAsync((void*)e->codec_dev, e->codec.data(), sizeof(float*) * m.n_codebooks, hipMemcpyHostToDevice, s));
    TRYC(dalloc(e, &e->proj_w, (size_t)m.p_d_model * m.d_embed));
    q3_launch_fill_f32(e->proj_w, (size_t)m.p_d_model * m.d_embed, seed, Q3_TID(Q3G_ASSET, 0, Q3WA_PROJ_W), 0.0f, 0.02f / Q3_IH4_STD, 1, s);
    TRYC(dalloc(e, &e->proj_b, (size_t)m.p_d_model));
    q3_launch_fill_f32(e->proj_b, m.p_d_model, seed, Q3_TID(Q3G_ASSET, 0, Q3WA_PROJ_B), 0.0f, 0.02f / Q3_IH4_STD, 0, s);
    e->tts_pad = e->text + (size_t)m.tts_pad_id * m.d_embed;
    }
    e->pproj.assign(m.n_codebooks, nullptr);
    for (int q = 0; q < m.n_codebooks; ++q) {
        const int rows = q == 0 ? m.codec0_rows : m.codecq_rows;
        TRYC(dalloc(e, &e->pproj[q], (size_t)rows * m.p_d_model));
        Q3Project pj{}; pj.x = e->codec[q]; pj.ldx = m.d_embed; pj.rows = rows; pj.w = e->proj_w; pj.bias = e->proj_b; pj.n_in = m.d_embed; pj.n_out = m.p_d_model;
        pj.y = e->pproj[q]; pj.ldy = m.p_d_model;
        q3_launch_project(pj, s);
    }
    HIPC(hipStreamSynchronize(s));
    TRYC(dalloc(e, &e->slots, (size_t)B));
    HIPC(hipHostMalloc((void**)&e->slots_host, sizeof(Q3Slot) * 2 * B, hipHostMallocDefault));
    memset(e->slots_host, 0, sizeof(Q3Slot) * 2 * B);
    TRYC(dalloc(e, &e->codes, (size_t)B * cfg->max_steps_cap * m.n_codebooks)); TRYC(dalloc(e, &e->rng, (size_t)B * cfg->max_steps_cap));
    {
        const int nb = B;
        const int nqkv_max = std::max(e->T.nqkv, e->P.nqkv), nq_max = std::max(e->T.nq, e->P.nq), F_max = std::max(e->T.F, e->P.F);
        e->lanes.resize(1);
        Q3Lane& L = e->lanes[0];
        L.nb = nb;
        HIPC(hipStreamCreateWithFlags(&L.stream, hipStreamNonBlocking));
        HIPC(hipEventCreate(&L.ev_begin)); HIPC(hipEventCreate(&L.ev_end));
        TRYC(dalloc(e, &L.xT, (size_t)nb * m.t_d_model)); TRYC(dalloc(e, &L.logits, (size_t)nb * m.t_vocab)); TRYC(dalloc(e, &L.logits_tmp, (size_t)nb * std::max(m.t_vocab, m.t_d_model)));
        TRYC(dalloc(e, &L.fb, (size_t)nb * m.d_embed));
        TRYC(dalloc(e, &L.px, (size_t)2 * nb * m.p_d_model)); TRYC(dalloc(e, &L.keys, (size_t)nb * (m.codebook_size / 16)));
        const size_t nb16 = ((size_t)nb + 15) & ~(size_t)15, nb2_16 = ((size_t)2 * nb + 15) & ~(size_t)15;
        TRYC(dalloc(e, &L.xbT, nb16 * m.t_d_model)); TRYC(dalloc(e, &L.sspT, (size_t)nb * (m.t_d_model / 16)));
        L.rt16T = (int)(nb16 / 16);
        if (e->T.a8) TRYC(dalloc(e, &L.ascT, nb16 * (m.t_d_model / 32)));
        TRYC(dalloc(e, &L.xbP, nb2_16 * m.p_d_model)); TRYC(dalloc(e, &L.sspP, (size_t)2 * nb * (m.p_d_model / 16)));
        TRYC(dalloc(e, &L.row_pos_t, (size_t)nb)); TRYC(dalloc(e, &L.slot_id, (size_t)nb)); TRYC(dalloc(e, &L.perm, (size_t)nb));
        TRYC(dalloc(e, &L.posA, (size_t)2 * nb)); TRYC(dalloc(e, &L.slotA, (size_t)2 * nb)); TRYC(dalloc(e, &L.pos_q, (size_t)m.n_codebooks * nb));
        std::vector<int> sid(nb), pa(2 * nb), sla(2 * nb), pq((size_t)m.n_codebooks * nb), rp(nb, -1);
        for (int b = 0; b < nb; ++b) { sid[b] = b; pa[b] = 0; pa[nb + b] = 1; sla[b] = sla[nb + b] = b; }
        for (int q = 0; q < m.n_codebooks; ++q) for (int b = 0; b < nb; ++b) pq[(size_t)q * nb + b] = q + 1;
        HIPC(hipMemcpyAsync(L.slot_id, sid.data(), nb * 4, hipMemcpyHostToDevice, s));
        HIPC(hipMemcpyAsync(L.posA, pa.data(), 2 * nb * 4, hipMemcpyHostToDevice, s));
        HIPC(hipMemcpyAsync(L.slotA, sla.data(), 2 * nb * 4, hipMemcpyHostToDevice, s));
        HIPC(hipMemcpyAsync(L.pos_q, pq.data(), pq.size() * 4, hipMemcpyHostToDevice, s));
        HIPC(hipMemcpyAsync(L.row_pos_t, rp.data(), nb * 4, hipMemcpyHostToDevice, s));
        HIPC(hipStreamSynchronize(s));
        TRYC(alloc_scratch(e, L.sc, 2 * nb, nqkv_max, nq_max, F_max, std::max(m.t_d_model, m.p_d_model)));
        for (int r = 1; r < nb && r < 16; r *= 2) e->buckets.push_back(r);
        for (int r = 16; r < nb; r += 16) e->buckets.push_back(r);
        e->buckets.push_back(nb);
        e->cur_bucket = (int)e->buckets.size() - 1;
        e->row_of_slot = sid; e->slot_of_row = sid;
    }
    TRYC(alloc_scratch(e, e->sc_pre, cfg->n_ctx, e->T.nqkv, e->T.nq, e->T.F, m.t_d_model));
    TRYC(dalloc(e, &e->xp, (size_t)cfg->n_ctx * m.t_d_model));
    TRYC(dalloc(e, &e->xbp, (((size_t)cfg->n_ctx + 15) & ~(size_t)15) * m.t_d_model)); TRYC(dalloc(e, &e->sspp, (size_t)cfg->n_ctx * (m.t_d_model / 16)));
    e->rt16p = (cfg->n_ctx + 15) / 16;
    if (e->T.a8) TRYC(dalloc(e, &e->ascp, (size_t)e->rt16p * 16 * (m.t_d_model / 32)));
    TRYC(dalloc(e, &e->pf_pos, (size_t)cfg->n_ctx)); TRYC(dalloc(e, &e->pf_slot, (size_t)cfg->n_ctx)); TRYC(dalloc(e, &e->pf_seg, (size_t)3 * cfg->max_batch));
    { std::vector<int> pp(cfg->n_ctx); for (int i = 0; i < cfg->n_ctx; ++i) pp[i] = i;
      HIPC(hipMemcpyAsync(e->pf_pos, pp.data(), pp.size() * 4, hipMemcpyHostToDevice, s)); HIPC(hipStreamSynchronize(s)); }
    e->prow_cap = cfg->n_ctx;
    TRYC(dalloc(e, &e->prow_dev, (size_t)e->prow_cap)); TRYC(dalloc(e, &e->spk_dev, (size_t)m.d_embed));
    TRYC(dalloc(e, &e->refcodes_dev, (size_t)cfg->n_ctx * 16));
    {
        TRYC(dalloc(e, &e->marker_row, (size_t)m.d_embed));
        const Q3PromptRow mr{1, m.tts_pad_id, 0, 0};
        HIPC(hipMemcpyAsync(e->prow_dev, &mr, sizeof(mr), hipMemcpyHostToDevice, s));
        HIPC(hipStreamSynchronize(s));
        q3_launch_prompt_rows(e->prow_dev, 1, e->text, m.text_vocab, e->codec_dev, m.codec0_rows, m.codecq_rows, m.n_codebooks, e->spk_dev, m.d_embed, e->marker_row, s);
        HIPC(hipStreamSynchronize(s));
    }
    if (cfg->with_vocoder) {
        TRYC(q3_voc_create(e));
        HIPC(hipHostMalloc((void**)&e->first_chunk_host, sizeof(float) * 4 * (size_t)q3_voc_samples_per_frame(e), hipHostMallocDefault));
    }
    HIPC(hipStreamSynchronize(s));
    if (!(getenv("Q3TTS_NO_GRAPH") && atoi(getenv("Q3TTS_NO_GRAPH")))) {
        Q3Lane& L = e->lanes[0];
        L.graphs.resize(e->buckets.size(), nullptr); L.execs.resize(e->buckets.size(), nullptr);
        for (size_t bi = 0; bi < e->buckets.size(); ++bi) {
            HIPC(hipStreamBeginCapture(L.stream, hipStreamCaptureModeThreadLocal));
            const int refused = record_frame(e, L, L.stream, e->buckets[bi]);
            HIPC(hipStreamEndCapture(L.stream, &L.graphs[bi]));
            if (refused) { q3_set_err(e, Q3TTS_ERR_INVALID, "frame step: " + std::to_string(refused) + " kernel launch(es) refused for this model shape"); return fail(Q3TTS_ERR_INVALID); }
            HIPC(hipGraphInstantiate(&L.execs[bi], L.graphs[bi], nullptr, nullptr, 0));
            HIPC(hipStreamSynchronize(L.stream));
        }
    }
    e->tm.algo_bytes_per_step = 0;
#undef TRYC
#undef HIPC
    *out = e;
    return Q3TTS_OK;
}

extern "C" void q3tts_engine_destroy(q3tts_engine* e) {
    if (!e) return;
    if (q3tts_session* ss = e->session.load()) q3tts_session_close(ss);
    hipSetDevice(e->cfg.device);
    if (e->stream) hipStreamSynchronize(e->stream);
    if (e->vstream) hipStreamSynchronize(e->vstream);
    if (e->voc) q3_voc_destroy(e);
    q3_mel_destroy(e);
    q3_clone_destroy(e);
    if (e->first_chunk_host) hipHostFree(e->first_chunk_host);
    for (auto& L : e->lanes) {
        if (L.stream) hipStreamSynchronize(L.stream);
        for (auto ge : L.execs) if (ge) hipGraphExecDestroy(ge);
        for (auto gr : L.graphs) if (gr) hipGraphDestroy(gr);
        hipFree(L.logits_tmp); hipFree(L.perm);
        hipFree(L.xT); hipFree(L.logits); hipFree(L.fb); hipFree(L.px); hipFree(L.keys);
        hipFree(L.xbT); hipFree(L.sspT); hipFree(L.xbP); hipFree(L.sspP); hipFree(L.ascT);
        hipFree(L.row_pos_t); hipFree(L.slot_id); hipFree(L.posA); hipFree(L.slotA); hipFree(L.pos_q);
        hipFree(L.sc.qkv); hipFree(L.sc.att); hipFree(L.sc.h); hipFree(L.sc.asc_att); hipFree(L.sc.asc_h);
        if (L.ev_begin) hipEventDestroy(L.ev_begin); if (L.ev_end) hipEventDestroy(L.ev_end);
        if (L.stream) hipStreamDestroy(L.stream);
    }
    free_tfm(e->T); free_tfm(e->P);
    hipFree(e->text); for (auto p : e->codec) hipFree(p); for (auto p : e->pproj) hipFree(p); hipFree((void*)e->codec_dev); hipFree(e->proj_w); hipFree(e->proj_b);
    hipFree(e->tts_pad_own); hipFree(e->marker_row); hipFree(e->dev_pcm);
    hipFree(e->slots); if (e->slots_host) hipHostFree(e->slots_host);
    hipFree(e->codes); hipFree(e->rng);
    hipFree(e->sc_pre.qkv); hipFree(e->sc_pre.att); hipFree(e->sc_pre.h); hipFree(e->sc_pre.asc_att); hipFree(e->sc_pre.asc_h); hipFree(e->ascp);
    hipFree(e->xp); hipFree(e->xbp); hipFree(e->sspp); hipFree(e->pf_pos); hipFree(e->pf_slot); hipFree(e->pf_seg); hipFree(e->prow_dev); hipFree(e->spk_dev); hipFree(e->refcodes_dev);
    for (auto ev : e->fin_ev) if (ev) hipEventDestroy(ev);
    for (auto ev : e->probe_ev) if (ev) hipEventDestroy(ev);
    if (e->ev0) hipEventDestroy(e->ev0); if (e->ev1) hipEventDestroy(e->ev1); if (e->ev2) hipEventDestroy(e->ev2); if (e->ev3) hipEventDestroy(e->ev3);
    if (e->stream) hipStreamDestroy(e->stream);
    if (e->vstream && e->vstream != e->stream) hipStreamDestroy(e->vstream);
    delete e;
}

extern "C" int q3tts_set_sampler(q3tts_engine* e, float temperature, int32_t top_k, float top_p, int32_t has_seed, uint64_t seed) {
    if (!e) return q3_set_err(nullptr, Q3TTS_ERR_INVALID, "null engine");
    Q3_NOT_IN_SESSION(e);
    e->temperature = temperature; e->top_k = top_k; e->top_p = top_p; e->has_seed = has_seed; e->seed = seed;
    return Q3TTS_OK;
}
extern "C" int q3tts_set_max_steps(q3tts_engine* e, int32_t n) {
    if (!e) return q3_set_err(nullptr, Q3TTS_ERR_INVALID, "null engine");
    Q3_NOT_IN_SESSION(e);
    if (n < 0 || n > e->cfg.max_steps_cap) return q3_set_err(e, Q3TTS_ERR_INVALID, "max_steps exceeds max_steps_cap");
    e->max_steps = n;
    return Q3TTS_OK;
}
extern "C" void q3tts_free(void* p) { free(p); }
extern "C" int q3tts_set_device_pcm(q3tts_engine* e, int32_t enable) {
    Q3_NOT_IN_SESSION(e);
    if (!e) return q3_set_err(nullptr, Q3TTS_ERR_INVALID, "null engine");
    e->dev_pcm_on = enable ? 1 : 0;
    return Q3TTS_OK;
}
extern "C" int q3tts_get_device_pcm(q3tts_engine* e, float** base, int64_t* stride_samples, int32_t* n_rows) {
    if (!e || !base || !stride_samples || !n_rows) return q3_set_err(e, Q3TTS_ERR_INVALID, "null argument");
    *base = e->dev_pcm; *stride_samples = (int64_t)e->dev_pcm_stride; *n_rows = e->dev_pcm_n;
    return Q3TTS_OK;
}

enum { PAD = 2148, BOS = 2149, THINK = 2154, NOTHINK = 2155, THINK_BOS = 2156, THINK_EOS = 2157, CODEC_BOS_ICL = 2160 };
enum { BOS_TOKEN = 151672, EOS_TOKEN = 151673 };

static int build_prompt_dev(q3tts_engine* e, const q3tts_prompt_desc* p, float* out, int max_rows, int* n_out) {
    const q3tts_model_config& m = e->cfg.model;
    if (!p || (p->n_text > 0 && !p->text_ids)) return q3_set_err(e, Q3TTS_ERR_INVALID, "prompt: text_ids missing");
    const int marker = m.tts_pad_id;
    std::vector<Q3PromptRow> rows;
    int ref_row0 = -1;
    auto T1 = [&](int id) { rows.push_back({1, id, 0, 0}); };
    auto MC = [&](int cid) { rows.push_back({1, marker, 2, cid}); };
    auto TP = [&](int tid) { rows.push_back({1, tid, 2, PAD}); };
    if (p->instruct_ids) {
        T1(151644); T1(872); T1(198);
        for (int i = 0; i < p->n_instruct; ++i) T1((int)p->instruct_ids[i]);
        T1(151645); T1(198);
    }
    T1(151644); T1(77091); T1(198);
    if (p->lang_id >= 0) { MC(THINK); MC(THINK_BOS); MC(p->lang_id); MC(THINK_EOS); }
    else { MC(NOTHINK); MC(THINK_BOS); MC(THINK_EOS); }
    if (p->spk_id >= 0) MC(p->spk_id);
    else if (p->spk_emb) rows.push_back({1, marker, -1, 0});
    if (p->ref_codes) {
        TP(BOS_TOKEN);
        for (int i = 0; i < p->n_ref_text; ++i) TP((int)p->ref_text_ids[i]);
        TP(EOS_TOKEN);
        MC(CODEC_BOS_ICL);
        ref_row0 = (int)rows.size();
        for (int i = 0; i < p->n_ref_frames; ++i) rows.push_back({-2, 0, 0, 0});
        MC(PAD);
    }
    TP(BOS_TOKEN);
    for (int i = 0; i < p->n_text; ++i) TP((int)p->text_ids[i]);
    TP(EOS_TOKEN);
    MC(BOS);
    const int n = (int)rows.size();
    if (n > max_rows || n > e->prow_cap) return q3_set_err(e, Q3TTS_ERR_INVALID, "prompt longer than n_ctx");
    hipStream_t s = e->stream;
    Q3_HIP(e, hipMemcpyAsync(e->prow_dev, rows.data(), sizeof(Q3PromptRow) * n, hipMemcpyHostToDevice, s));
    if (p->spk_emb) Q3_HIP(e, hipMemcpyAsync(e->spk_dev, p->spk_emb, (size_t)m.d_embed * 4, hipMemcpyHostToDevice, s));
    Q3_HIP(e, hipStreamSynchronize(s));
    q3_launch_prompt_rows(e->prow_dev, n, e->text, m.text_vocab, e->codec_dev, m.codec0_rows, m.codecq_rows, m.n_codebooks, e->spk_dev,
                          m.d_embed, out, s);
    if (ref_row0 >= 0 && p->n_ref_frames > 0) {
        Q3_HIP(e, hipMemcpyAsync(e->refcodes_dev, p->ref_codes, (size_t)p->n_ref_frames * 16 * 4, hipMemcpyHostToDevice, s));
        Q3_HIP(e, hipStreamSynchronize(s));
        q3_launch_prompt_ref_frames(e->refcodes_dev, p->n_ref_frames, e->marker_row, e->codec_dev, m.codec0_rows,
                                    m.codecq_rows, m.n_codebooks, m.d_embed, out + (size_t)ref_row0 * m.d_embed, s);
    }
    *n_out = n;
    return Q3TTS_OK;
}

extern "C" int q3tts_build_prompt(q3tts_engine* e, const q3tts_prompt_desc* p, float** out_embd, int32_t* out_n) {
    Q3_NOT_IN_SESSION(e);
    if (!e || !p || !out_embd || !out_n) return q3_set_err(e, Q3TTS_ERR_INVALID, "null argument");
    Q3_HIP(e, hipSetDevice(e->cfg.device));
    int n = 0;
    TRY(build_prompt_dev(e, p, e->xp, e->cfg.n_ctx, &n));
    const size_t bytes = (size_t)n * e->cfg.model.d_embed * 4;
    float* h = (float*)malloc(bytes);
    if (!h) return q3_set_err(e, Q3TTS_ERR_OOM, "malloc");
    hipError_t er = hipMemcpyAsync(h, e->xp, bytes, hipMemcpyDeviceToHost, e->stream);
    if (er == hipSuccess) er = hipStreamSynchronize(e->stream);
    if (er != hipSuccess) { free(h); return q3_set_err(e, Q3TTS_ERR_DEVICE, hipGetErrorString(er)); }
    *out_embd = h; *out_n = n;
    return Q3TTS_OK;
}

static int plan_rows(q3tts_engine* e, const std::vector<int>& live_in) {
    Q3Lane& L = e->lanes[0];
    const int B = e->B;
    std::vector<int> live(live_in);
    std::sort(live.begin(), live.end());
    int bi = 0;
    while (bi + 1 < (int)e->buckets.size() && e->buckets[bi] < (int)live.size()) ++bi;
    bool ok = bi == e->cur_bucket;
    if (ok) for (int b : live) if (e->row_of_slot[b] >= e->buckets[bi]) { ok = false; break; }
    if (ok) return Q3TTS_OK;
    std::vector<int> slot_of_row(B, -1), perm(B), used(B, 0), sla(2 * (size_t)B, 0), pa(2 * (size_t)B, 0);
    int r = 0;
    for (int b : live) { slot_of_row[r++] = b; used[b] = 1; }
    for (int b = 0; b < B && r < B; ++b) if (!used[b]) slot_of_row[r++] = b;
    const int bs = e->buckets[bi];
    for (r = 0; r < B; ++r) perm[r] = e->row_of_slot[slot_of_row[r]];
    for (r = 0; r < bs; ++r) { sla[r] = sla[bs + r] = slot_of_row[r]; pa[bs + r] = 1; }
    hipStream_t s = e->stream;
    Q3_HIP(e, hipMemcpyAsync(L.perm, perm.data(), (size_t)B * 4, hipMemcpyHostToDevice, s));
    Q3_HIP(e, hipMemcpyAsync(L.slot_id, slot_of_row.data(), (size_t)B * 4, hipMemcpyHostToDevice, s));
    Q3_HIP(e, hipMemcpyAsync(L.slotA, sla.data(), (size_t)2 * B * 4, hipMemcpyHostToDevice, s));
    Q3_HIP(e, hipMemcpyAsync(L.posA, pa.data(), (size_t)2 * B * 4, hipMemcpyHostToDevice, s));
    q3_launch_gather_rows(L.logits_tmp, L.logits, L.perm, B, e->cfg.model.t_vocab, s);
    Q3_HIP(e, hipMemcpyAsync(L.logits, L.logits_tmp, (size_t)B * e->cfg.model.t_vocab * 4, hipMemcpyDeviceToDevice, s));
    q3_launch_gather_rows(L.logits_tmp, L.xT, L.perm, B, e->cfg.model.t_d_model, s);
    Q3_HIP(e, hipMemcpyAsync(L.xT, L.logits_tmp, (size_t)B * e->cfg.model.t_d_model * 4, hipMemcpyDeviceToDevice, s));
    Q3_HIP(e, hipStreamSynchronize(s));
    for (r = 0; r < B; ++r) e->row_of_slot[slot_of_row[r]] = r;
    e->slot_of_row = slot_of_row;
    e->cur_bucket = bi;
    return Q3TTS_OK;
}

static double now_ms();
static int run_chunk(q3tts_engine* e, int CH, float* dev_ms) {
    hipStream_t s = e->stream;
    Q3Lane& L = e->lanes[0];
    const double hp0 = now_ms();
    Q3_HIP(e, hipEventRecord(e->ev1, s));
    Q3_HIP(e, hipStreamWaitEvent(L.stream, e->ev1, 0));
    Q3_HIP(e, hipEventRecord(L.ev_begin, L.stream));
    e->probe_i = 0;
    if (e->probe) { hipEventRecord(e->probe_ev[8], L.stream); hipEventRecord(e->probe_ev[9], L.stream); }
    for (int i = 0; i < CH; ++i) {
        if (!L.execs.empty() && !e->probe) { Q3_HIP(e, hipGraphLaunch(L.execs[e->cur_bucket], L.stream)); }
        else {
            if (record_frame(e, L, L.stream, e->buckets[e->cur_bucket])) return q3_set_err(e, Q3TTS_ERR_INVALID, "frame step: a kernel launch was refused for this model shape");
            Q3_HIP(e, hipGetLastError());
        }
    }
    e->row_steps += (long long)CH * e->buckets[e->cur_bucket];
    Q3_HIP(e, hipEventRecord(L.ev_end, L.stream));
    Q3_HIP(e, hipStreamWaitEvent(s, L.ev_end, 0));
    Q3_HIP(e, hipEventRecord(e->ev3, s));
    Q3_HIP(e, hipMemcpyAsync(e->slots_host, e->slots, sizeof(Q3Slot) * e->B, hipMemcpyDeviceToHost, s));
    const double hp1 = now_ms();
    Q3_HIP(e, hipStreamSynchronize(s));
    e->hp_launch += hp1 - hp0; e->hp_sync += now_ms() - hp1;
    if (dev_ms) { *dev_ms = 0.0f; hipEventElapsedTime(dev_ms, L.ev_begin, L.ev_end); }
    for (int i = 0; i + 1 < e->probe_i; i += 2) {
        float ms = 0.0f;
        if (hipEventElapsedTime(&ms, e->probe_ev[i], e->probe_ev[i + 1]) == hipSuccess) { e->probe_ms += ms; ++e->probe_cnt; }
    }
    if (e->probe) {
        float ms = 0.0f;
        if (hipEventElapsedTime(&ms, e->probe_ev[8], e->probe_ev[9]) == hipSuccess) { e->probe_empty_ms += ms; ++e->probe_empty_cnt; }
    }
    return Q3TTS_OK;
}

static uint64_t wall_seed() {
    return (uint64_t)std::chrono::duration_cast<std::chrono::nanoseconds>(std::chrono::system_clock::now().time_since_epoch()).count();
}

struct Adm { int b; const q3tts_request* r; int n, row0, max_steps; };

static int admit_group(q3tts_engine* e, std::vector<Adm>& grp, int total) {
    const q3tts_model_config& m = e->cfg.model;
    hipStream_t s = e->stream;
    if (grp.empty()) return Q3TTS_OK;
    std::vector<int> pos(total), slot(total);
    for (const Adm& a : grp) for (int i = 0; i < a.n; ++i) { pos[a.row0 + i] = i; slot[a.row0 + i] = a.b; }
    Q3_HIP(e, hipMemcpyAsync(e->pf_pos, pos.data(), (size_t)total * 4, hipMemcpyHostToDevice, s));
    Q3_HIP(e, hipMemcpyAsync(e->pf_slot, slot.data(), (size_t)total * 4, hipMemcpyHostToDevice, s));
    std::vector<int> seg; int seg_max = 0;
    for (const Adm& a : grp) { seg.push_back(a.row0); seg.push_back(a.n); seg.push_back(a.b); seg_max = std::max(seg_max, a.n); }
    Q3_HIP(e, hipMemcpyAsync(e->pf_seg, seg.data(), seg.size() * 4, hipMemcpyHostToDevice, s));
    Q3_HIP(e, hipStreamSynchronize(s));
    if (e->T.a8) q3_launch_norm_inputs_q8(e->xp, m.t_d_model, total, m.t_d_model, e->T.attn_norm[0], (int8_t*)e->xbp, e->ascp, e->rt16p, e->sspp, m.t_d_model / 16, s);
    else q3_launch_norm_inputs(e->xp, m.t_d_model, total, m.t_d_model, e->T.attn_norm[0], e->xbp, 0, e->sspp, m.t_d_model / 16, s);
    const int rl = run_layers(e, e->T, e->xp, e->xbp, e->sspp, total, e->pf_pos, e->pf_slot, e->sc_pre, s, false, nullptr, 0, 0, e->pf_seg, (int)grp.size(), seg_max, e->ascp, e->rt16p);
    if (rl) return q3_set_err(e, Q3TTS_ERR_INVALID, "prefill: a kernel launch was refused for this model shape");
    Q3_HIP(e, hipGetLastError());
    for (const Adm& a : grp) {
        const q3tts_request* r = a.r;
        const int b = a.b;
        Q3Lane& L = e->lanes[0];
        const int row = e->row_of_slot[b];
        q3_launch_copy_rows(L.xT + (size_t)row * m.t_d_model, m.t_d_model, e->xp + (size_t)(a.row0 + a.n - 1) * m.t_d_model, m.t_d_model, 1, m.t_d_model, s);
        const size_t lastr = (size_t)(a.row0 + a.n - 1);
        Q3BGemm g{}; g.a = e->xbp; g.a_row0 = (int)lastr; g.B = 1; g.w = e->T.head; g.wscale = e->T.q8 ? e->T.shead : nullptr; g.K = m.t_d_model; g.N = m.t_vocab;
        g.ssp = e->sspp + lastr * (m.t_d_model / 16); g.ld_ssp = m.t_d_model / 16; g.ntiles = m.t_d_model / 16; g.d_norm = m.t_d_model; g.eps = m.rms_eps;
        g.epi = Q3_EPI_STORE; g.y = L.logits + (size_t)row * m.t_vocab; g.ldy = m.t_vocab;
        if (e->T.a8) { g.ascale = e->ascp; g.a_rt16 = e->rt16p; }
        if (e->T.a8 ? q3_launch_bgemm8(g, s) : q3_launch_bgemm(g, s)) return q3_set_err(e, Q3TTS_ERR_INVALID, "prefill head: launch refused for this model shape");
        float temperature = e->temperature, top_p = e->top_p; int top_k = e->top_k, has_seed = e->has_seed; uint64_t seed = e->seed;
        if (!r->use_engine_sampler) { temperature = r->temperature; top_k = r->top_k; top_p = r->top_p; has_seed = r->has_seed; seed = r->seed; }
        if (!has_seed) seed = wall_seed();
        if (temperature > 0.0f) {
            std::vector<float> draws(a.max_steps);
            q3_stdrng_f32(seed, a.max_steps, draws.data());
            Q3_HIP(e, hipMemcpyAsync(e->rng + (size_t)b * e->cfg.max_steps_cap, draws.data(), (size_t)a.max_steps * 4, hipMemcpyHostToDevice, s));
            Q3_HIP(e, hipStreamSynchronize(s));
        }
        Q3Slot* st = e->slots_host + e->B + b;
        memset(st, 0, sizeof(*st));
        st->active = 1; st->cur_pos = a.n; st->n_frames = 0; st->max_steps = a.max_steps; st->min_frames = r->min_frames;
        st->force_eos_at = r->force_eos_at; st->top_k = top_k; st->temperature = temperature; st->top_p = top_p;
        st->rng_base = b * e->cfg.max_steps_cap;
        Q3_HIP(e, hipMemcpyAsync(e->slots + b, st, sizeof(Q3Slot), hipMemcpyHostToDevice, s));
        if (e->voc) TRY(q3_voc_reset(e, b));
    }
    return Q3TTS_OK;
}

static int admit_many(q3tts_engine* e, const int* slots, const q3tts_request* const* reqs, int count, int* rc) {
    const q3tts_model_config& m = e->cfg.model;
    hipStream_t s = e->stream;
    std::vector<Adm> grp;
    int total = 0;
    for (int i = 0; i < count; ++i) {
        const q3tts_request* r = reqs[i];
        rc[i] = Q3TTS_OK;
        const int max_steps = r->max_steps > 0 ? r->max_steps : e->max_steps;
        if (max_steps > e->cfg.max_steps_cap) { rc[i] = q3_set_err(e, Q3TTS_ERR_INVALID, "max_steps exceeds max_steps_cap"); continue; }
        int n = 0;
        for (int attempt = 0; attempt < 2; ++attempt) {
            const int room = e->cfg.n_ctx - total;
            if (r->prompt_embd) {
                n = r->n_tok;
                if (n <= 0 || n > e->cfg.n_ctx) { rc[i] = q3_set_err(e, Q3TTS_ERR_INVALID, "n_tok out of range"); break; }
                if (n > room) { if (total == 0) { rc[i] = q3_set_err(e, Q3TTS_ERR_INVALID, "n_tok out of range"); break; } }
                else { Q3_HIP(e, hipMemcpyAsync(e->xp + (size_t)total * m.d_embed, r->prompt_embd, (size_t)n * m.d_embed * 4, hipMemcpyHostToDevice, s)); break; }
            } else if (r->prompt) {
                const int brc = build_prompt_dev(e, r->prompt, e->xp + (size_t)total * m.d_embed, room, &n);
                if (brc == Q3TTS_OK) break;
                if (total == 0) { rc[i] = brc; break; }
            } else { rc[i] = q3_set_err(e, Q3TTS_ERR_INVALID, "request has neither prompt_embd nor prompt"); break; }
            TRY(admit_group(e, grp, total));
            grp.clear(); total = 0;
        }
        if (rc[i] != Q3TTS_OK) continue;
        if (n + max_steps > e->cfg.n_ctx) { rc[i] = q3_set_err(e, Q3TTS_ERR_INVALID, "prompt + max_steps exceeds n_ctx"); continue; }
        grp.push_back(Adm{slots[i], r, n, total, max_steps});
        total += n;
    }
    return admit_group(e, grp, total);
}

static int admit(q3tts_engine* e, int b, const q3tts_request* r) {
    int rc = Q3TTS_OK;
    int st = admit_many(e, &b, &r, 1, &rc);
    return st != Q3TTS_OK ? st : rc;
}

static double now_ms() {
    return std::chrono::duration<double, std::milli>(std::chrono::steady_clock::now().time_since_epoch()).count();
}

struct SlotRun { int req = -1; double t_first = 0; };

int q3_voc_dispatch(q3tts_engine* e, const char* live, const char* want, int* voc_frames, bool more, bool* first) {
    const int B = e->B;
    hipStream_t vs = e->vstream;
    bool waited = false;
    *first = false;
    auto ensure_wait = [&]() -> int { if (!waited) { Q3_HIP(e, hipStreamWaitEvent(vs, e->ev3, 0)); waited = true; } return Q3TTS_OK; };
    int list[64], real[64];
    for (;;) {
        int ns = 0;
        for (int b = 0; b < B; ++b) {
            if (!live[b] || !want[b]) continue;
            const int pend = e->slots_host[b].n_frames - voc_frames[b];
            if (pend >= 4 || (pend > 0 && !e->slots_host[b].active)) { real[ns] = std::min(pend, 4); list[ns++] = b; }
        }
        if (!ns) break;
        TRY(ensure_wait());
        int still = 0;
        for (int b = 0; b < B; ++b) if (live[b] && e->slots_host[b].active) ++still;
        TRY(q3_voc_decode_batch(e, list, real, ns, 4, vs, (still > 0 || more) ? 1 : 0));
        for (int i = 0; i < ns; ++i) { if (voc_frames[list[i]] == 0) *first = true; voc_frames[list[i]] += real[i]; }
    }
    for (int b = 0; b < B; ++b)
        if (live[b] && !e->slots_host[b].active && (e->cfg.vocoder_flush_tail || e->slots_host[b].n_frames % 4 != 0)) q3_voc_mark_last(e, b);
    return Q3TTS_OK;
// ... 848 lines not shown
```

### qwen3-tts-rust_amd/csrc/q3_kernels.h

```cpp
#pragma once
#include "q3_common.h"

enum { Q3_EPI_STORE = 0, Q3_EPI_RESID = 1, Q3_EPI_SWIGLU = 2, Q3_EPI_ARGMAX = 3, Q3_EPI_GELU = 4 };

#ifdef Q3_STAMPS
#define Q3_STAMP_FIELD unsigned long long* dbg;
#define Q3_STAMP(p, i) do { if ((p).dbg && threadIdx.x == 0) (p).dbg[((size_t)blockIdx.x + (size_t)gridDim.x * blockIdx.y) * 8 + (i)] = __builtin_amdgcn_s_memrealtime(); } while (0)
#else
#define Q3_STAMP_FIELD
#define Q3_STAMP(p, i) do { } while (0)
#endif

#include <mutex>
struct Q3PerDevice {
    std::mutex mu; size_t have[64] = {0};
    template <class F> void ensure(size_t want, F set_attr) {
        int dev = 0; if (hipGetDevice(&dev) != hipSuccess) dev = 0;
        std::lock_guard<std::mutex> lk(mu);
        if (have[dev & 63] < want) { set_attr(); have[dev & 63] = want; }
    }
};

struct Q3Gemm {
    const float* x; int ldx; int B;
    const uint4* w; int K, N;
    const float* norm_w; float eps;
    const float* bias;
    float* y; int ldy;
    unsigned long long* keys; int key_stride;
    int epi;
#ifdef Q3_STAMPS
    unsigned long long* dbg;
#endif
};
void q3_launch_gemm(const Q3Gemm& g, hipStream_t s);
Q3_HD size_t q3_atile_off(int row, int k, int kblocks) {
    const int c = k & 31;
    return ((((size_t)(row >> 4) * kblocks + (k >> 5)) * 64 + ((c & 15) >> 2) * 16 + (row & 15)) << 3) + (c & 3) + ((c & 16) >> 2);
}
Q3_HD size_t q3_q8_off(int row, int k, int kpairs) {
    const int c = k & 31;
    return ((((size_t)(row >> 4) * kpairs + (k >> 6)) * 64 + ((c & 15) >> 2) * 16 + (row & 15)) << 4) + ((k >> 5) & 1) * 8 + (c & 3) + ((c & 16) >> 2);
}
Q3_HD size_t q3_q8_scale_idx(int row, int kb, int rt16) {
    return ((((size_t)(kb >> 1) * rt16 + (row >> 4)) * 4 + ((row & 15) >> 2)) << 3) + (kb & 1) * 4 + (row & 3);
}
struct Q3BGemm {
    const uint16_t* a; int a_row0; int B;
    const uint4* w; int K, N;
    int w_once;
    const float* ssp; int ld_ssp; int ntiles; int d_norm; float eps;
    int epi;
    float* y; int ldy;
    uint16_t* yb;
    const float* nw_next; float* ssp_out; int ld_ssp_out;
    const float* col_scale;
    const float* bias; int bias_n;
    int seg_rows; size_t seg_stride;
    unsigned long long* keys; int key_stride;
    const uint16_t* wscale;
    const uint16_t* ascale; int a_rt16; uint16_t* yscale; int y_rt16;
    Q3_STAMP_FIELD
};
int q3_launch_bgemm(const Q3BGemm& g, hipStream_t s);
int q3_launch_bgemm8(const Q3BGemm& g, hipStream_t s);
void q3_bgemm8_pick(const Q3BGemm& g, int* rt, int* nt);
void q3_bgemm_pick(const Q3BGemm& g, int* rt, int* nt, int* d, int* ntw, int* big);
void q3_bgemm_force(int rt, int nt);
void q3_bgemm_prepare();
void q3_bgemm_big_policy(int policy);
void q3_launch_norm_inputs(const float* x, int ldx, int rows, int d, const float* nw, uint16_t* xb, int xb_row0, float* ssp, int ld_ssp, hipStream_t s);
void q3_launch_norm_inputs_q8(const float* x, int ldx, int rows, int d, const float* nw, int8_t* xq, uint16_t* xscale, int rt16, float* ssp, int ld_ssp, hipStream_t s);
struct Q3Project {
    const float* x; int ldx; int rows;
    const float* w; const float* bias; int n_in, n_out;
    float* y; int ldy;
    const float* nw; uint16_t* xb; float* ssp; int ld_ssp;
    const float* norm_w; float eps;
};
int q3_launch_project(const Q3Project& p, hipStream_t s);
#define Q3_LDS_BARRIER() do { asm volatile("s_waitcnt lgkmcnt(0)" ::: "memory"); __builtin_amdgcn_s_barrier(); asm volatile("" ::: "memory"); } while (0)
#ifdef __HIPCC__
__device__ __forceinline__ void q3_row_map(int row, const int* row_pos, const int* row_slot, int slot_mod, int pos_const, int* pos, int* slot) {
    if (slot_mod > 0) { *slot = row % slot_mod; *pos = pos_const + row / slot_mod; }
    else { *pos = row_pos[row]; *slot = *pos < 0 ? 0 : row_slot[row]; }
}
__device__ __forceinline__ void q3_norm_out(float v, float nwv, uint16_t* xb_elem, float* ssp_tile, bool tile_leader) {
    *xb_elem = q3_bf16(v * nwv);
    float sq = v * v;
    sq = sq + __shfl_xor(sq, 1); sq = sq + __shfl_xor(sq, 2); sq = sq + __shfl_xor(sq, 4); sq = sq + __shfl_xor(sq, 8);
    if (tile_leader) *ssp_tile = sq;
}
#endif

#ifdef __HIPCC__
__device__ __forceinline__ void q3_q8_out32(float v, int row, int k, int kpairs, int rt16, int8_t* q, uint16_t* sc) {
    float amax = fabsf(v);
#pragma unroll
    for (int m = 1; m <= 16; m <<= 1) amax = fmaxf(amax, __shfl_xor(amax, m));
    const float d = amax / 127.0f, id = d != 0.0f ? 1.0f / d : 0.0f;
    q[q3_q8_off(row, k, kpairs)] = (int8_t)(int)roundf(v * id);
    if ((k & 31) == 0) sc[q3_q8_scale_idx(row, k >> 5, rt16)] = __builtin_bit_cast(unsigned short, (_Float16)d);
}
__device__ __forceinline__ void q3_q8_out2x16(float v0, float v1, int row, int k0, int kpairs, int rt16, int8_t* q, uint16_t* sc) {
    float amax = fmaxf(fabsf(v0), fabsf(v1));
#pragma unroll
    for (int m = 1; m <= 8; m <<= 1) amax = fmaxf(amax, __shfl_xor(amax, m));
    const float d = amax / 127.0f, id = d != 0.0f ? 1.0f / d : 0.0f;
    q[q3_q8_off(row, k0, kpairs)] = (int8_t)(int)roundf(v0 * id);
    q[q3_q8_off(row, k0 + 1, kpairs)] = (int8_t)(int)roundf(v1 * id);
    if ((k0 & 31) == 0) sc[q3_q8_scale_idx(row, k0 >> 5, rt16)] = __builtin_bit_cast(unsigned short, (_Float16)d);
}
__device__ __forceinline__ void q3_q8_out8x4(const float* v, int row, int k0, int kpairs, int rt16, int8_t* q, uint16_t* sc, bool store) {
    float amax = 0.0f;
#pragma unroll
    for (int i = 0; i < 8; ++i) amax = fmaxf(amax, fabsf(v[i]));
    amax = fmaxf(amax, __shfl_xor(amax, 1)); amax = fmaxf(amax, __shfl_xor(amax, 2));
    const float d = amax / 127.0f, id = d != 0.0f ? 1.0f / d : 0.0f;
    if (store) {
#pragma unroll
        for (int i = 0; i < 8; ++i) q[q3_q8_off(row, k0 + i, kpairs)] = (int8_t)(int)roundf(v[i] * id);
        if ((k0 & 31) == 0) sc[q3_q8_scale_idx(row, k0 >> 5, rt16)] = __builtin_bit_cast(unsigned short, (_Float16)d);
    }
}
#endif

struct Q3Fill {
    uint4* dst; int N, K;
    int mode;
    int row0, rows;
    uint32_t tid_a, tid_b;
    const uint16_t* src_a; const uint16_t* src_b;
    uint64_t seed; float scale;
    uint16_t* dst_scale; const uint8_t* src8_a; const uint8_t* src8_b;
};
void q3_launch_fill_tiled(const Q3Fill& f, hipStream_t s);
void q3_launch_fill_tiled_q8(const Q3Fill& f, hipStream_t s);
void q3_launch_fill_f32(float* dst, size_t n, uint64_t seed, uint32_t tid, float base, float scale, int round_bf16, hipStream_t s);

struct Q3QkPrep {
    float* qkv; int ld; int rows;
    int Hq, Hkv, hd;
    const float* qnw; const float* knw; float eps;
    const float* cs; const float* sn;
    uint16_t* kc; uint16_t* vc; int n_ctx;
    const int* row_pos; const int* row_slot;
    int slot_mod, pos_const;
};
void q3_launch_qk_prep(const Q3QkPrep& a, hipStream_t s);

struct Q3Attend {
    const float* qkv; int ld; int rows;
    float* out; int ldo;
    int out_bf16;
    uint16_t* out_scale; int out_rt16;
    int Hq, Hkv, hd;
    const uint16_t* kc; const uint16_t* vc; int n_ctx;
    const int* row_pos; const int* row_slot;
    int slot_mod, pos_const;
    int fused;
    Q3QkPrep prep;
    const int* seg; int n_seg; int seg_max_n;
    Q3_STAMP_FIELD
};
void q3_launch_attend(const Q3Attend& a, hipStream_t s);
void q3_attend_policy(int decode, int prefill);

struct Q3Sample {
    float* logits; int ld; int limit; int eos;
    Q3Slot* slots; int B;
    const int* row_slot;
    const float* rng;
    int* codes; int max_steps_cap; int ncb;
};
void q3_launch_sample(const Q3Sample& a, hipStream_t s);
void q3_launch_sample_rows(const float* logits, int n, int ld, int limit, float temperature, int top_k, float top_p,
                           const float* r, int* out, hipStream_t s);

struct Q3PredInput {
    const float* xT; const float* out_norm; float eps; int d;
    const float* codec0; int codec0_rows;
    const float* pproj0; const float* proj_b; int dp;
    const Q3Slot* slots; const int* row_slot; float* X; float* px; float* fb; int B;
    const float* nw; uint16_t* xb; float* ssp;
};
void q3_launch_pred_input(const Q3PredInput& a, hipStream_t s);
int q3_launch_sample_input(const Q3Sample& a, const Q3PredInput& p, const Q3Project& pj, hipStream_t s);

struct Q3PredNext {
    const unsigned long long* keys; int n_key_parts; int q; int ncb;
    const float* codec_q; int rows_q; int d;
    Q3Slot* slots; const int* row_slot; int B;
    int* codes; int max_steps_cap;
    float* fb; const float* tts_pad; float* xT; int* row_pos_t;
    const float* pproj_q; const float* proj_b; int dp; float* px;
    const float* nw; uint16_t* xb; float* ssp;
    uint16_t* xscale; int x_rt16;
    Q3_STAMP_FIELD
};
void q3_launch_pred_next(const Q3PredNext& a, hipStream_t s);

struct Q3PromptRow { int32_t kindA, idA, kindB, idB; };
void q3_launch_prompt_rows(const Q3PromptRow* rows, int n, const float* text, int text_vocab, const float* const* codec,
                           int codec0_rows, int codecq_rows, int ncb, const float* spk, int d, float* out, hipStream_t s);
void q3_launch_prompt_ref_frames(const int* codes, int n_frames, const float* marker, const float* const* codec,
                                 int codec0_rows, int codecq_rows, int ncb, int d, float* out, hipStream_t s);

void q3_launch_copy_rows(float* dst, int ldd, const float* src, int lds, int rows, int cols, hipStream_t s);

void q3_launch_gather_rows(float* dst, const float* src, const int* perm, int rows, int cols, hipStream_t s);
void q3_launch_rmsnorm_rows(const float* x, int ldx, const float* w, float eps, int d, int rows, float* out, int ldo, hipStream_t s);

#define Q3_PCM_MAX_ENT 64
struct Q3PcmEnt { int32_t row, first, count, pad; long long dst_off; };
struct Q3PcmPack { Q3PcmEnt e[Q3_PCM_MAX_ENT]; };
void q3_launch_pcm_pack(const float* src, size_t stride, const Q3PcmPack& ents, int n_ent, int max_count, int i16, void* dst, hipStream_t s);
```

### qwen3-tts-rust_amd/csrc/q3_kernels.hip

```cpp
#include "q3_kernels.h"

#define WAVE 64

typedef unsigned int u32x4 __attribute__((ext_vector_type(4)));
__device__ __forceinline__ uint4 ntload16(const uint4* p) {
    const u32x4 v = __builtin_nontemporal_load((const u32x4*)p);
    return make_uint4(v.x, v.y, v.z, v.w);
}

__device__ __forceinline__ float wave_sum(float v) {
#pragma unroll
    for (int m = 32; m >= 1; m >>= 1) v = v + __shfl_xor(v, m);
    return v;
}
__device__ __forceinline__ float wave_max(float v) {
#pragma unroll
    for (int m = 32; m >= 1; m >>= 1) v = fmaxf(v, __shfl_xor(v, m));
    return v;
}


__global__ void k_fill_tiled(Q3Fill f, int nb0, int nb_count) {
    const size_t gid = (size_t)blockIdx.x * blockDim.x + threadIdx.x;
    const int kblocks = f.K >> 5;
// ... 885 lines not shown
    const int tid = threadIdx.x;
    __shared__ unsigned long long wbest[4];
    if (temperature <= 0.0f) {
        unsigned long long best = 0;
        for (int i = tid; i < limit; i += 256) { const unsigned long long k = q3_argmax_key(logits[i], (uint32_t)i); best = k > best ? k : best; }
#pragma unroll
        for (int m = 32; m >= 1; m >>= 1) { const unsigned long long o = __shfl_xor(best, m); best = o > best ? o : best; }
        if ((tid & 63) == 0) wbest[tid >> 6] = best;
        __syncthreads();
        unsigned long long b = wbest[0];
        for (int w = 1; w < 4; ++w) b = wbest[w] > b ? wbest[w] : b;
        __syncthreads();
        return q3_argmax_idx(b);
    }
    bool select = top_k_i > 0 && top_k_i <= 256 && top_k_i < limit;
    if (select) {
        __shared__ unsigned long long lm[256];
        __shared__ unsigned long long thr_s;
        __shared__ int n_sel;
        unsigned long long* sel = (unsigned long long*)probs;
        unsigned long long loc[SAMP_MAX / 256];
        unsigned long long lmax = 0;
#pragma unroll
        for (int j = 0; j < SAMP_MAX / 256; ++j) { const int i = tid + j * 256; loc[j] = i < limit ? q3_argmax_key(logits[i], (uint32_t)i) : 0ull; lmax = loc[j] > lmax ? loc[j] : lmax; }
        lm[tid] = lmax;
        if (tid == 0) { thr_s = 0ull; n_sel = 0; }
        __syncthreads();
        int cnt = 0;
        for (int j = 0; j < 256; ++j) cnt += lm[j] > lmax ? 1 : 0;
        if (cnt == top_k_i - 1 && lmax != 0ull) thr_s = lmax;
        __syncthreads();
        const unsigned long long T = thr_s;
#pragma unroll
        for (int j = 0; j < SAMP_MAX / 256; ++j)
            if (loc[j] != 0ull && loc[j] >= T) { const int pos = atomicAdd(&n_sel, 1); if (pos < SAMP_MAX / 2) sel[pos] = loc[j]; }
        __syncthreads();
        const int n = n_sel;
        if (n > SAMP_MAX / 2) select = false;
        else {
            for (int i = tid; i < top_k_i; i += 256) keys[i] = 0ull;
            __syncthreads();
            for (int i = tid; i < n; i += 256) {
                const unsigned long long mine = sel[i];
                int rank = 0;
                for (int j = 0; j < n; ++j) rank += sel[j] > mine ? 1 : 0;
                if (rank < top_k_i) keys[rank] = mine;
            }
        }
        __syncthreads();
    }
    int NP = 64;
    while (NP < limit) NP <<= 1;
    if (!select) {
    for (int i = tid; i < NP; i += 256) keys[i] = i < limit ? q3_argmax_key(logits[i], (uint32_t)i) : 0ull;
    __syncthreads();
    }
    for (int k = 2; !select && k <= NP; k <<= 1)
        for (int j = k >> 1; j > 0; j >>= 1) {
            for (int i = tid; i < NP; i += 256) {
                const int ixj = i ^ j;
                if (ixj > i) {
                    const unsigned long long x = keys[i], y = keys[ixj];
                    const bool desc = (i & k) == 0;
                    if (desc ? (x < y) : (x > y)) { keys[i] = y; keys[ixj] = x; }
                }
            }
            __syncthreads();
        }
    __shared__ int result;
    int n_all = limit;
    {
        const size_t top_k = (size_t)(long long)top_k_i;
        if (top_k > 0 && top_k < (size_t)n_all) n_all = (int)top_k;
    }
    {
        const float max_logit = n_all > 0 ? q3_key_value(keys[0]) : 0.0f;
        for (int i = tid; i < n_all; i += 256) probs[i] = q3_expf((q3_key_value(keys[i]) - max_logit) / temperature);
    }
    __syncthreads();
    __shared__ float bc_s; __shared__ int cut_s;
    int n = n_all;
    if (tid == 0) { float sum = 0.0f; for (int i = 0; i < n; ++i) sum += probs[i]; bc_s = sum; }
    __syncthreads();
    { const float sum = bc_s; if (sum > 0.0f) for (int i = tid; i < n; i += 256) probs[i] /= sum; }
    __syncthreads();
    if (top_p < 1.0f) {
        if (tid == 0) {
            float cum = 0.0f; int cutoff = n;
            for (int i = 0; i < n; ++i) { cum += probs[i]; if (cum >= top_p) { cutoff = i + 1; break; } }
            float ns = 0.0f;
            for (int i = 0; i < cutoff; ++i) ns += probs[i];
            cut_s = cutoff; bc_s = ns;
        }
        __syncthreads();
        n = cut_s;
        { const float ns = bc_s; if (ns > 0.0f) for (int i = tid; i < n; i += 256) probs[i] /= ns; }
        __syncthreads();
    }
    if (tid == 0) {
        float cum = 0.0f; int res = -1;
        for (int i = 0; i < n; ++i) { cum += probs[i]; if (r < cum) { res = q3_argmax_idx(keys[i]); break; } }
        if (res < 0) res = n > 0 ? q3_argmax_idx(keys[0]) : 0;
        result = res;
    }
    __syncthreads();
    const int res = result;
    __syncthreads();
    return res;
}

__device__ int sample_frame(const Q3Sample& a, int b, unsigned long long* keys, float* probs) {
    const int tid = threadIdx.x, slot = a.row_slot[b];
    Q3Slot* sl = a.slots + slot;
    if (!sl->active) return -1;
    const int step = sl->n_frames;
    if (step >= sl->max_steps) {
        __syncthreads();
        if (tid == 0) sl->active = 0;
        return -1;
    }
    float* lg = a.logits + (size_t)b * a.ld;
    int code0;
    if (sl->force_eos_at >= 0 && step == sl->force_eos_at) code0 = a.eos;
    else {
        if (step < sl->min_frames && a.eos < a.limit) { if (tid == 0) lg[a.eos] = -INFINITY; }
        __syncthreads();
        const float temperature = sl->temperature;
        const float r = temperature > 0.0f ? a.rng[sl->rng_base + step] : 0.0f;
        code0 = sample_row(lg, a.limit, temperature, sl->top_k, sl->top_p, r, keys, probs);
    }
    __syncthreads();
    if (tid == 0) {
        if (code0 == a.eos) { sl->hit_eos = 1; sl->active = 0; }
        else { a.codes[((size_t)slot * a.max_steps_cap + step) * a.ncb] = code0; sl->code0 = code0; }
    }
    return code0 == a.eos ? -1 : code0;
}
__global__ __launch_bounds__(256) void k_sample(Q3Sample a) {
    __shared__ unsigned long long keys[SAMP_MAX];
    __shared__ float probs[SAMP_MAX];
    sample_frame(a, blockIdx.x, keys, probs);
}
void q3_launch_sample(const Q3Sample& a, hipStream_t s) { hipLaunchKernelGGL(k_sample, dim3(a.B), dim3(256), 0, s, a); }

__global__ __launch_bounds__(256) void k_sample_rows(const float* logits, int ld, int limit, float temperature, int top_k,
                                                     float top_p, const float* r, int* out) {
    __shared__ unsigned long long keys[SAMP_MAX];
    __shared__ float probs[SAMP_MAX];
    const int b = blockIdx.x;
    const int id = sample_row(logits + (size_t)b * ld, limit, temperature, top_k, top_p, r ? r[b] : 0.0f, keys, probs);
    if (threadIdx.x == 0) out[b] = id;
}
void q3_launch_sample_rows(const float* logits, int n, int ld, int limit, float temperature, int top_k, float top_p,
                           const float* r, int* out, hipStream_t s) {
    hipLaunchKernelGGL(k_sample_rows, dim3(n), dim3(256), 0, s, logits, ld, limit, temperature, top_k, top_p, r, out);
}

__device__ void pred_input_row(const Q3PredInput& a, int b, int code0) {
    __shared__ float rinv_s;
    const int tid = threadIdx.x, d = a.d;
    const float* x = a.xT + (size_t)b * d;
    const bool wantX = a.X != nullptr;
    if (wantX && tid < 64) {
        float acc = 0.0f;
        for (int c = tid; c < (d >> 2); c += 64) {
            const float4 v = ((const float4*)x)[c];
            acc = fmaf(v.x, v.x, acc); acc = fmaf(v.y, v.y, acc); acc = fmaf(v.z, v.z, acc); acc = fmaf(v.w, v.w, acc);
        }
        acc = wave_sum(acc);
        if (tid == 0) rinv_s = 1.0f / sqrtf(acc / (float)d + a.eps);
    }
    __syncthreads();
    const float rinv = wantX ? rinv_s : 0.0f;
    const bool ok = code0 >= 0 && code0 < a.codec0_rows;
    const float* e = a.codec0 + (size_t)(ok ? code0 : 0) * d;
    const float* pr = ok ? a.pproj0 + (size_t)code0 * a.dp : a.proj_b;
    constexpr int NI = 8, NP = 4;
    for (int i0 = 0; i0 < d; i0 += NI * 256) {
        float xv[NI], nv[NI], ev[NI];
#pragma unroll
        for (int u = 0; u < NI; ++u) {
            const int i = min(i0 + tid + u * 256, d - 1);
            xv[u] = wantX ? x[i] : 0.0f; nv[u] = wantX ? a.out_norm[i] : 0.0f; ev[u] = ok ? e[i] : 0.0f;
        }
#pragma unroll
        for (int u = 0; u < NI; ++u) {
            const int i = i0 + tid + u * 256;
            if (i < d) { if (wantX) a.X[(size_t)b * d + i] = (xv[u] * rinv) * nv[u]; a.fb[(size_t)b * d + i] = 0.0f + ev[u]; }
        }
    }
    const int r1 = a.B + b;
    for (int i0 = 0; i0 < a.dp; i0 += NP * 256) {
        float pv[NP], wv[NP];
#pragma unroll
        for (int u = 0; u < NP; ++u) { const int i = min(i0 + tid + u * 256, a.dp - 1); pv[u] = pr[i]; wv[u] = a.nw[i]; }
#pragma unroll
        for (int u = 0; u < NP; ++u) {
            const int i = i0 + tid + u * 256;
            if (i < a.dp) {
                a.px[(size_t)r1 * a.dp + i] = pv[u];
                q3_norm_out(pv[u], wv[u], a.xb + q3_atile_off(r1, i, a.dp >> 5), a.ssp + (size_t)r1 * (a.dp >> 4) + (i >> 4), (i & 15) == 0);
            }
        }
    }
}
__global__ __launch_bounds__(256) void k_pred_input(Q3PredInput a) {
    const Q3Slot* sl = a.slots + a.row_slot[blockIdx.x];
    if (!sl->active) return;
    pred_input_row(a, blockIdx.x, sl->code0);
}
void q3_launch_pred_input(const Q3PredInput& a, hipStream_t s) { hipLaunchKernelGGL(k_pred_input, dim3(a.B), dim3(256), 0, s, a); }

constexpr int PJ_KC = 64, PJ_LD = PJ_KC + 4, PJ_LDS_FLOATS = 4 * 16 * PJ_LD;
__device__ void project_tile(const Q3Project& p, int bx, int by, float* lds) {
    constexpr int KC = PJ_KC, LD = PJ_LD;
    float* ws = lds; float* xs = lds + 2 * 16 * LD;
    __shared__ float rinv16[16];
    const int tid = threadIdx.x, oc = tid & 15, rr = tid >> 4;
    const int o = bx * 16 + oc, row = by * 16 + rr;
    const float* wsrc = p.w + (size_t)(bx * 16 + rr) * p.n_in + 4 * oc;
    const float* xsrc = p.x + (size_t)min(by * 16 + rr, p.rows - 1) * p.ldx + 4 * oc;
    const float* nsrc = p.norm_w ? p.norm_w + 4 * oc : nullptr;
    float sum = p.bias[o];
    const int nch = p.n_in / KC;
    float4 wv = *(const float4*)wsrc, xv = *(const float4*)xsrc, nv = nsrc ? *(const float4*)nsrc : float4{1.0f, 1.0f, 1.0f, 1.0f};
    float rinv = 1.0f;
    if (nsrc) {
        const int wave = tid >> 6, lane = tid & 63;
        const float4* xr[4];
#pragma unroll
        for (int u = 0; u < 4; ++u) xr[u] = (const float4*)(p.x + (size_t)min(by * 16 + wave * 4 + u, p.rows - 1) * p.ldx);
        float acc[4] = {0.0f, 0.0f, 0.0f, 0.0f};
        for (int c = lane; c < (p.n_in >> 2); c += 64) {
            float4 v[4];
#pragma unroll
            for (int u = 0; u < 4; ++u) v[u] = xr[u][c];
#pragma unroll
            for (int u = 0; u < 4; ++u) { acc[u] = fmaf(v[u].x, v[u].x, acc[u]); acc[u] = fmaf(v[u].y, v[u].y, acc[u]); acc[u] = fmaf(v[u].z, v[u].z, acc[u]); acc[u] = fmaf(v[u].w, v[u].w, acc[u]); }
        }
#pragma unroll
        for (int u = 0; u < 4; ++u) { const float t = wave_sum(acc[u]); if (lane == 0) rinv16[wave * 4 + u] = 1.0f / sqrtf(t / (float)p.n_in + p.eps); }
        __syncthreads();
        rinv = rinv16[rr];
    }
    for (int c = 0; c < nch; ++c) {
        float* wl = ws + (c & 1) * 16 * LD; float* xl = xs + (c & 1) * 16 * LD;
        if (nsrc) { xv.x = (xv.x * rinv) * nv.x; xv.y = (xv.y * rinv) * nv.y; xv.z = (xv.z * rinv) * nv.z; xv.w = (xv.w * rinv) * nv.w; }
        *(float4*)(wl + rr * LD + 4 * oc) = wv; *(float4*)(xl + rr * LD + 4 * oc) = xv;
        if (c + 1 < nch) {
            wv = *(const float4*)(wsrc + (c + 1) * KC); xv = *(const float4*)(xsrc + (c + 1) * KC);
            if (nsrc) nv = *(const float4*)(nsrc + (c + 1) * KC);
        }
        __syncthreads();
        const float* wr = wl + oc * LD; const float* xr = xl + rr * LD;
#pragma unroll
        for (int k = 0; k < KC; k += 4) {
            const float4 a = *(const float4*)(xr + k), w4 = *(const float4*)(wr + k);
            sum += a.x * w4.x; sum += a.y * w4.y; sum += a.z * w4.z; sum += a.w * w4.w;
        }
    }
    const bool live = row < p.rows;
    if (live) p.y[(size_t)row * p.ldy + o] = sum;
    if (p.nw) {
        uint16_t hb = q3_bf16(sum * p.nw[o]);
        float sq = sum * sum;
        sq = sq + __shfl_xor(sq, 1); sq = sq + __shfl_xor(sq, 2); sq = sq + __shfl_xor(sq, 4); sq = sq + __shfl_xor(sq, 8);
        if (live) {
            p.xb[q3_atile_off(row, o, p.n_out >> 5)] = hb;
            if (oc == 0) p.ssp[(size_t)row * p.ld_ssp + (o >> 4)] = sq;
        }
    }
}
__global__ __launch_bounds__(256) void k_project(Q3Project p) {
    __shared__ __attribute__((aligned(16))) float lds[PJ_LDS_FLOATS];
    project_tile(p, blockIdx.x, blockIdx.y, lds);
}
static bool project_ok(const Q3Project& p) { return p.rows >= 1 && p.n_out % 16 == 0 && p.n_in % 64 == 0 && p.ldx % 4 == 0; }
int q3_launch_project(const Q3Project& p, hipStream_t s) {
    if (!project_ok(p)) return -1;
    hipLaunchKernelGGL(k_project, dim3(p.n_out / 16, (p.rows + 15) / 16), dim3(256), 0, s, p);
    return 0;
}

static_assert(PJ_LDS_FLOATS * sizeof(float) <= SAMP_MAX * sizeof(unsigned long long), "the projection tile stages through the sampler's key array");
__global__ __launch_bounds__(256) void k_sample_input(Q3Sample a, Q3PredInput p, Q3Project pj) {
    __shared__ __attribute__((aligned(16))) unsigned long long keys[SAMP_MAX];
    __shared__ float probs[SAMP_MAX];
    if ((int)blockIdx.x >= a.B) {
        const int t = blockIdx.x - a.B, nx = pj.n_out >> 4;
        project_tile(pj, t % nx, t / nx, (float*)keys);
        return;
    }
    const int code0 = sample_frame(a, blockIdx.x, keys, probs);
    if (code0 < 0) return;
    pred_input_row(p, blockIdx.x, code0);
}
int q3_launch_sample_input(const Q3Sample& a, const Q3PredInput& p, const Q3Project& pj, hipStream_t s) {
    if (!project_ok(pj) || !pj.norm_w) return -1;
    hipLaunchKernelGGL(k_sample_input, dim3(a.B + (pj.n_out / 16) * ((pj.rows + 15) / 16)), dim3(256), 0, s, a, p, pj);
    return 0;
}

__global__ __launch_bounds__(256) void k_pred_next(Q3PredNext a) {
    const int b = blockIdx.x, tid = threadIdx.x, d = a.d;
    unsigned long long kk = tid < a.n_key_parts ? a.keys[(size_t)b * a.n_key_parts + tid] : 0ull;
    const int slot = a.row_slot[b];
    Q3Slot* sl = a.slots + slot;
    const bool last = a.q == a.ncb - 1;
    if (!sl->active) {
        if (last && tid == 0) a.row_pos_t[b] = -1;
        return;
    }
    __shared__ unsigned long long kmax_s[4];
    for (int t = tid + 256; t < a.n_key_parts; t += 256) { const unsigned long long o = a.keys[(size_t)b * a.n_key_parts + t]; kk = o > kk ? o : kk; }
#pragma unroll
    for (int m = 32; m >= 1; m >>= 1) { const unsigned long long o = __shfl_xor(kk, m); kk = o > kk ? o : kk; }
    if ((tid & 63) == 0) kmax_s[tid >> 6] = kk;
    __syncthreads();
    kk = kmax_s[0];
#pragma unroll
    for (int w = 1; w < 4; ++w) kk = kmax_s[w] > kk ? kmax_s[w] : kk;
    const int code = q3_argmax_idx(kk);
    const bool ok = code >= 0 && code < a.rows_q;
    const float* e = a.codec_q + (size_t)(ok ? code : 0) * d;
    const int frame = sl->n_frames;
    if (tid == 0) a.codes[((size_t)slot * a.max_steps_cap + frame) * a.ncb + a.q] = code;
    constexpr int NI = 8, NP = 4;
    const float* pr = ok ? a.pproj_q + (size_t)code * a.dp : a.proj_b;
    float pv[NP], wv[NP];
    if (!last) {
#pragma unroll
        for (int u = 0; u < NP; ++u) { const int i = min(tid + u * 256, a.dp - 1); pv[u] = pr[i]; wv[u] = a.nw[i]; }
    }
    for (int i0 = 0; i0 < d; i0 += NI * 256) {
        float ev[NI], fv[NI], tp[NI], nv[NI];
#pragma unroll
        for (int u = 0; u < NI; ++u) {
            const int i = min(i0 + tid + u * 256, d - 1);
            ev[u] = ok ? e[i] : 0.0f; fv[u] = a.fb[(size_t)b * d + i];
            if (last) { tp[u] = a.tts_pad[i]; nv[u] = a.nw[i]; }
        }
#pragma unroll
        for (int u = 0; u < NI; ++u) {
            const int i = i0 + tid + u * 256;
            if (i >= d) continue;
            float f = fv[u] + ev[u];
            if (!last) a.fb[(size_t)b * d + i] = f;
            else {
                f = f + tp[u]; a.xT[(size_t)b * d + i] = f;
                if (a.xscale) {
                    q3_q8_out32(f * nv[u], b, i, d >> 6, a.x_rt16, (int8_t*)a.xb, a.xscale);
                    float sq = f * f;
                    sq = sq + __shfl_xor(sq, 1); sq = sq + __shfl_xor(sq, 2); sq = sq + __shfl_xor(sq, 4); sq = sq + __shfl_xor(sq, 8);
                    if ((i & 15) == 0) a.ssp[(size_t)b * (d >> 4) + (i >> 4)] = sq;
                } else
                q3_norm_out(f, nv[u], a.xb + q3_atile_off(b, i, d >> 5), a.ssp + (size_t)b * (d >> 4) + (i >> 4), (i & 15) == 0);
            }
        }
    }
    if (!last) {
#pragma unroll
        for (int u = 0; u < NP; ++u) {
            const int i = tid + u * 256;
            if (i < a.dp) {
                a.px[(size_t)b * a.dp + i] = pv[u];
                q3_norm_out(pv[u], wv[u], a.xb + q3_atile_off(b, i, a.dp >> 5), a.ssp + (size_t)b * (a.dp >> 4) + (i >> 4), (i & 15) == 0);
            }
        }
        for (int i = tid + NP * 256; i < a.dp; i += 256) {
            const float v = pr[i];
            a.px[(size_t)b * a.dp + i] = v;
            q3_norm_out(v, a.nw[i], a.xb + q3_atile_off(b, i, a.dp >> 5), a.ssp + (size_t)b * (a.dp >> 4) + (i >> 4), (i & 15) == 0);
        }
    }
    if (last) {
        __syncthreads();
        if (tid == 0) { a.row_pos_t[b] = sl->cur_pos; sl->cur_pos = sl->cur_pos + 1; sl->n_frames = frame + 1; }
    }
}
void q3_launch_pred_next(const Q3PredNext& a, hipStream_t s) { hipLaunchKernelGGL(k_pred_next, dim3(a.B), dim3(256), 0, s, a); }

__device__ __forceinline__ float prompt_elem(int kind, int id, int i, const float* text, int text_vocab,
                                             const float* const* codec, int codec0_rows, int codecq_rows, int ncb,
                                             const float* spk, int d) {
    if (kind == 1) {
        if (id >= 0 && id < text_vocab) return text[(size_t)id * d + i];
        return fmodf((float)((unsigned long long)id * 17ull + (unsigned long long)i), 2.0f) - 1.0f;
    }
    if (kind >= 2) {
        const int q = kind - 2;
        const int rows = q == 0 ? codec0_rows : codecq_rows;
        if (id < 0) id = 0;
        if (q < ncb && id < rows) return codec[q][(size_t)id * d + i];
        return 0.0f;
    }
    if (kind == -1) return spk[i];
    return 0.0f;
}
__global__ void k_prompt_rows(const Q3PromptRow* rows, const float* text, int text_vocab, const float* const* codec,
                              int codec0_rows, int codecq_rows, int ncb, const float* spk, int d, float* out) {
    const Q3PromptRow r = rows[blockIdx.x];
    for (int i = threadIdx.x; i < d; i += blockDim.x) {
        const float a = prompt_elem(r.kindA, r.idA, i, text, text_vocab, codec, codec0_rows, codecq_rows, ncb, spk, d);
        float v = a;
        if (r.kindB != 0) v = a + prompt_elem(r.kindB, r.idB, i, text, text_vocab, codec, codec0_rows, codecq_rows, ncb, spk, d);
        out[(size_t)blockIdx.x * d + i] = v;
    }
}
void q3_launch_prompt_rows(const Q3PromptRow* rows, int n, const float* text, int text_vocab, const float* const* codec,
                           int codec0_rows, int codecq_rows, int ncb, const float* spk, int d, float* out, hipStream_t s) {
    hipLaunchKernelGGL(k_prompt_rows, dim3(n), dim3(256), 0, s, rows, text, text_vocab, codec, codec0_rows, codecq_rows, ncb, spk, d, out);
}
__global__ void k_prompt_ref_frames(const int* codes, const float* marker, const float* const* codec, int codec0_rows,
                                    int codecq_rows, int ncb, int d, float* out) {
    const int f = blockIdx.x;
    for (int i = threadIdx.x; i < d; i += blockDim.x) {
        float sum = 0.0f;
        for (int q = 0; q < 16; ++q)
            sum += prompt_elem(2 + q, codes[f * 16 + q], i, nullptr, 0, codec, codec0_rows, codecq_rows, ncb, nullptr, d);
        out[(size_t)f * d + i] = marker[i] + sum;
    }
}
void q3_launch_prompt_ref_frames(const int* codes, int n_frames, const float* marker, const float* const* codec,
                                 int codec0_rows, int codecq_rows, int ncb, int d, float* out, hipStream_t s) {
    hipLaunchKernelGGL(k_prompt_ref_frames, dim3(n_frames), dim3(256), 0, s, codes, marker, codec, codec0_rows, codecq_rows, ncb, d, out);
}

__global__ void k_copy_rows(float* dst, int ldd, const float* src, int lds, int cols) {
    const int r = blockIdx.x;
    for (int i = threadIdx.x; i < cols; i += blockDim.x) dst[(size_t)r * ldd + i] = src[(size_t)r * lds + i];
}
__global__ void k_gather_rows(float* dst, const float* src, const int* perm, int cols) {
    const int r = blockIdx.y;
    const float* sp = src + (size_t)perm[r] * cols;
    for (int i = blockIdx.x * blockDim.x + threadIdx.x; i < cols; i += gridDim.x * blockDim.x) dst[(size_t)r * cols + i] = sp[i];
}
void q3_launch_gather_rows(float* dst, const float* src, const int* perm, int rows, int cols, hipStream_t s) {
    hipLaunchKernelGGL(k_gather_rows, dim3((cols + 255) / 256, rows), dim3(256), 0, s, dst, src, perm, cols);
}
void q3_launch_copy_rows(float* dst, int ldd, const float* src, int lds, int rows, int cols, hipStream_t s) {
    hipLaunchKernelGGL(k_copy_rows, dim3(rows), dim3(256), 0, s, dst, ldd, src, lds, cols);
}

template <int CPL>
__global__ __launch_bounds__(256) void k_rmsnorm_rows(const float* x, int ldx, const float* w, float eps, int d, int rows, float* out, int ldo) {
    const int r = blockIdx.x * 4 + (threadIdx.x >> 6), lane = threadIdx.x & 63;
    if (r >= rows) return;
    const float4* xr = (const float4*)(x + (size_t)r * ldx);
    float4* orow = (float4*)(out + (size_t)r * ldo);
    const float4* w4 = (const float4*)w;
    if constexpr (CPL > 0) {
        float4 v[CPL], g[CPL];
#pragma unroll
        for (int i = 0; i < CPL; ++i) { v[i] = xr[lane + 64 * i]; g[i] = w4[lane + 64 * i]; }
        float acc = 0.0f;
#pragma unroll
        for (int i = 0; i < CPL; ++i) { acc = fmaf(v[i].x, v[i].x, acc); acc = fmaf(v[i].y, v[i].y, acc); acc = fmaf(v[i].z, v[i].z, acc); acc = fmaf(v[i].w, v[i].w, acc); }
        acc = wave_sum(acc);
        const float rinv = 1.0f / sqrtf(acc / (float)d + eps);
#pragma unroll
        for (int i = 0; i < CPL; ++i)
            orow[lane + 64 * i] = make_float4((v[i].x * rinv) * g[i].x, (v[i].y * rinv) * g[i].y, (v[i].z * rinv) * g[i].z, (v[i].w * rinv) * g[i].w);
    } else {
        float acc = 0.0f;
        for (int c = lane; c < (d >> 2); c += 64) {
            const float4 v = xr[c];
            acc = fmaf(v.x, v.x, acc); acc = fmaf(v.y, v.y, acc); acc = fmaf(v.z, v.z, acc); acc = fmaf(v.w, v.w, acc);
        }
        acc = wave_sum(acc);
        const float rinv = 1.0f / sqrtf(acc / (float)d + eps);
        for (int c = lane; c < (d >> 2); c += 64) {
            const float4 v = xr[c], g = w4[c];
            orow[c] = make_float4((v.x * rinv) * g.x, (v.y * rinv) * g.y, (v.z * rinv) * g.z, (v.w * rinv) * g.w);
        }
    }
}
void q3_launch_rmsnorm_rows(const float* x, int ldx, const float* w, float eps, int d, int rows, float* out, int ldo, hipStream_t s) {
    dim3 grid((rows + 3) / 4);
    if (d == 2048) hipLaunchKernelGGL((k_rmsnorm_rows<8>), grid, dim3(256), 0, s, x, ldx, w, eps, d, rows, out, ldo);
    else if (d == 1024) hipLaunchKernelGGL((k_rmsnorm_rows<4>), grid, dim3(256), 0, s, x, ldx, w, eps, d, rows, out, ldo);
    else if (d == 512) hipLaunchKernelGGL((k_rmsnorm_rows<2>), grid, dim3(256), 0, s, x, ldx, w, eps, d, rows, out, ldo);
    else hipLaunchKernelGGL((k_rmsnorm_rows<0>), grid, dim3(256), 0, s, x, ldx, w, eps, d, rows, out, ldo);
}

__device__ __forceinline__ void pcm_put(float* d, float v) { *d = v; }
__device__ __forceinline__ void pcm_put(int16_t* d, float v) {
    v = v * 32767.0f;
    v = fminf(fmaxf(v, -32768.0f), 32767.0f);
    *d = (int16_t)(int)truncf(v);
}
template <typename T>
__global__ __launch_bounds__(256) void k_pcm_pack(const float* __restrict__ src, size_t stride, const Q3PcmPack ents, T* __restrict__ dst) {
    const Q3PcmEnt en = ents.e[blockIdx.y];
    const int n = en.count;
    if (n <= 0) return;
    const float* s = src + (size_t)en.row * stride + en.first;
    T* d = dst + en.dst_off;
    const int head = min(n, (int)((4 - (((uintptr_t)s >> 2) & 3)) & 3));
    const int nv = (n - head) >> 2;
    const int tid = blockIdx.x * blockDim.x + threadIdx.x, nth = gridDim.x * blockDim.x;
    if (tid < head) pcm_put(d + tid, s[tid]);
    const float4* sv = (const float4*)(s + head);
    for (int i = tid; i < nv; i += nth) {
        const float4 v = sv[i];
        T* o = d + head + 4 * i;
        pcm_put(o, v.x); pcm_put(o + 1, v.y); pcm_put(o + 2, v.z); pcm_put(o + 3, v.w);
    }
    for (int i = head + 4 * nv + tid; i < n; i += nth) pcm_put(d + i, s[i]);
}
void q3_launch_pcm_pack(const float* src, size_t stride, const Q3PcmPack& ents, int n_ent, int max_count, int i16, void* dst, hipStream_t s) {
    if (n_ent <= 0) return;
    const int gx = std::max(1, std::min(64, (max_count / 4 + 255) / 256));
    if (i16) hipLaunchKernelGGL(k_pcm_pack<int16_t>, dim3(gx, n_ent), dim3(256), 0, s, src, stride, ents, (int16_t*)dst);
    else hipLaunchKernelGGL(k_pcm_pack<float>, dim3(gx, n_ent), dim3(256), 0, s, src, stride, ents, (float*)dst);
}
```

Measured before the change: 674.4.

## Fold predictor argmax and next-input prep into the first QKV GEMM

For codebook steps after the first, the separate pred_next kernel is replaced by a fused path inside the layer-0 QKV bgemm. That path reduces the argmax keys, gathers A-operand tiles from a precomputed table, and performs the fb, px and codes updates in its epilogue. A new init-time kernel builds, per codebook, bf16 rows of the projected embedding table already multiplied by the attention norm weight, plus per-row RMS scales. This removes one kernel launch and the RMSNorm pass per step on the latency-bound predictor loop. In exchange it costs extra memory, restricts the GEMM to NT=1 tiles, and spreads the side-effect writes redundantly across workgroups.

After: 680.2, median of 6. Within noise of the previous version (+0.9%).

```diff
diff --git a/qwen3-tts-rust_amd/csrc/q3_bgemm.hip b/qwen3-tts-rust_amd/csrc/q3_bgemm.hip
--- a/qwen3-tts-rust_amd/csrc/q3_bgemm.hip
+++ b/qwen3-tts-rust_amd/csrc/q3_bgemm.hip
@@ -26,8 +26,131 @@
 }
 __device__ __forceinline__ float bg_f16(uint32_t bits) { return (float)__builtin_bit_cast(_Float16, (unsigned short)bits); }
 
+template <int RT>
+struct BgFold {
+    static constexpr int NR = 2 * RT;
+    unsigned long long k0[NR], k1[NR];
+    int rs[5], act[5], nfr;
+    float fbv[2], cdv[2], pxv[2], sc[NR];
+    bool okc[2];
+    int e0, stride, nrow;
+
+    __device__ __forceinline__ void phase1(const Q3BGemm& g, int row0, int cg, int wave, int lane) {
+        const auto& f = g.fold;
+        nrow = min(RT * 16, g.B - row0); stride = (int)gridDim.x * 512; e0 = cg * 512 + (int)threadIdx.x;
+        const int tf = nrow * f.d, tpx = nrow * g.K;
+#pragma unroll
+        for (int u = 0; u < 2; ++u) {
+            rs[u] = f.row_slot[row0 + min(e0 + u * stride, tf - 1) / f.d];
+            rs[2 + u] = f.row_slot[row0 + min(e0 + u * stride, tpx - 1) / g.K];
+        }
+        rs[4] = f.row_slot[row0 + min(lane, nrow - 1)];
+#pragma unroll
+        for (int i = 0; i < NR; ++i) {
+            const unsigned long long* kp = f.keys + (size_t)min(row0 + wave + 8 * i, g.B - 1) * f.n_key_parts;
+            k0[i] = kp[min(lane, f.n_key_parts - 1)];
+            k1[i] = kp[min(lane + 64, f.n_key_parts - 1)];
+        }
+    }
+    template <int D>
+    __device__ __forceinline__ void phase2(const Q3BGemm& g, int row0, int wave, int lane, int kq, int r, int per, int kb0, int* scode, u32x4 (&aq)[D][RT]) {
+        const auto& f = g.fold;
+#pragma unroll
+        for (int u = 0; u < 5; ++u) act[u] = f.slots[rs[u]].active;
+        nfr = f.slots[rs[4]].n_frames;
+#pragma unroll
+        for (int i = 0; i < NR; ++i) {
+            unsigned long long kk = k1[i] > k0[i] ? k1[i] : k0[i];
+#pragma unroll
+            for (int m = 32; m >= 1; m >>= 1) { const unsigned long long o = __shfl_xor(kk, m); kk = o > kk ? o : kk; }
+            if (lane == 0) scode[wave + 8 * i] = q3_argmax_idx(kk);
+        }
+        Q3_LDS_BARRIER();
+        const int kblocks = g.K >> 5, lmax = nrow - 1;
+        auto trow = [&](int code) { return code >= 0 && code < f.rows_q ? code : f.rows_q; };
+        const u32x4* xt = (const u32x4*)f.xtab;
+#pragma unroll
+        for (int i = 0; i < RT; ++i) {
+            const size_t tb = ((size_t)trow(scode[min(16 * i + r, lmax)]) * kblocks + kb0) * 4 + kq;
+#pragma unroll
+            for (int s = 0; s < D; ++s) aq[s][i] = xt[tb + (size_t)min(s, per - 1) * 4];
+        }
+        const int tf = nrow * f.d, tpx = nrow * g.K;
+#pragma unroll
+        for (int u = 0; u < 2; ++u) {
+            const int e = min(e0 + u * stride, tf - 1), rl = e / f.d, c = e - rl * f.d, code = scode[rl];
+            okc[u] = code >= 0 && code < f.rows_q;
+            fbv[u] = f.fb[(size_t)(row0 + rl) * f.d + c];
+            cdv[u] = f.codec[(size_t)(okc[u] ? code : 0) * f.d + c];
+            const int ep = min(e0 + u * stride, tpx - 1), rp = ep / g.K, cp = ep - rp * g.K, codep = scode[rp];
+            pxv[u] = ((codep >= 0 && codep < f.rows_q) ? f.table + (size_t)codep * g.K : f.proj_b)[cp];
+        }
+#pragma unroll
+        for (int i = 0; i < NR; ++i) sc[i] = f.stab[trow(scode[min(wave + 8 * i, lmax)])];
+    }
+    __device__ __forceinline__ void phase3(const Q3BGemm& g, int row0, int cg, int wave, int lane, const int* scode, float* srow) {
+        const auto& f = g.fold;
+        if (lane == 0) {
+#pragma unroll
+            for (int i = 0; i < NR; ++i) srow[wave + 8 * i] = sc[i];
+        }
+        const int tf = nrow * f.d, tpx = nrow * g.K;
+#pragma unroll
+        for (int u = 0; u < 2; ++u) {
+            const int e = e0 + u * stride;
+            if (e < tf && act[u]) { const int rl = e / f.d; f.fb[(size_t)(row0 + rl) * f.d + (e - rl * f.d)] = fbv[u] + (okc[u] ? cdv[u] : 0.0f); }
+            if (e < tpx && act[2 + u]) { const int rp = e / g.K; f.px[(size_t)(row0 + rp) * g.K + (e - rp * g.K)] = pxv[u]; }
+        }
+        if (cg == 0 && wave == 0 && lane < nrow && act[4]) f.codes[((size_t)rs[4] * f.max_steps_cap + nfr) * f.ncb + f.q] = scode[lane];
+        for (int e = e0 + 2 * stride; e < max(tf, tpx); e += stride) {
+            if (e < tf) {
+                const int rl = e / f.d, c = e - rl * f.d, code = scode[rl];
+                if (f.slots[f.row_slot[row0 + rl]].active)
+                    f.fb[(size_t)(row0 + rl) * f.d + c] = f.fb[(size_t)(row0 + rl) * f.d + c] + ((code >= 0 && code < f.rows_q) ? f.codec[(size_t)code * f.d + c] : 0.0f);
+            }
+            if (e < tpx) {
+                const int rp = e / g.K, cp = e - rp * g.K, code = scode[rp];
+                if (f.slots[f.row_slot[row0 + rp]].active)
+                    f.px[(size_t)(row0 + rp) * g.K + cp] = (code >= 0 && code < f.rows_q) ? f.table[(size_t)code * g.K + cp] : f.proj_b[cp];
+            }
+        }
+    }
+};
+
+__global__ __launch_bounds__(64) void k_fold_table(const float* table, int rows, const float* proj_b, const float* nw, int K, float eps, u32x4* xtab, float* stab) {
+    const int row = blockIdx.x, lane = threadIdx.x, nt = K >> 4;
+    const float* v = row < rows ? table + (size_t)row * K : proj_b;
+    for (int fi = lane; fi < (K >> 5) * 4; fi += 64) {
+        const int c = (fi >> 2) * 32 + (fi & 3) * 4;
+        uint16_t h[8];
+#pragma unroll
+        for (int k = 0; k < 4; ++k) { h[k] = q3_bf16(v[c + k] * nw[c + k]); h[4 + k] = q3_bf16(v[c + 16 + k] * nw[c + 16 + k]); }
+        u32x4 o;
+        o.x = h[0] | ((uint32_t)h[1] << 16); o.y = h[2] | ((uint32_t)h[3] << 16); o.z = h[4] | ((uint32_t)h[5] << 16); o.w = h[6] | ((uint32_t)h[7] << 16);
+        xtab[(size_t)row * (K >> 5) * 4 + fi] = o;
+    }
+    auto tile = [&](int t) {
+        float q[4];
+#pragma unroll
+        for (int k = 0; k < 4; ++k) {
+            const float* p = v + t * 16 + 4 * k;
+            q[k] = (p[0] * p[0] + p[1] * p[1]) + (p[2] * p[2] + p[3] * p[3]);
+        }
+        return (q[0] + q[1]) + (q[2] + q[3]);
+    };
+    float a = lane < nt ? tile(lane) : 0.0f;
+    const float a1 = lane + 64 < nt ? tile(lane + 64) : 0.0f;
+    if (lane + 64 < nt) a = a + a1;
+#pragma unroll
+    for (int m = 32; m >= 1; m >>= 1) a = a + __shfl_xor(a, m);
+    if (lane == 0) stab[row] = 1.0f / sqrtf(a / (float)K + eps);
+}
+void q3_launch_fold_table(const float* table, int rows, const float* proj_b, const float* nw, int K, float eps, uint4* xtab, float* stab, hipStream_t s) {
+    hipLaunchKernelGGL(k_fold_table, dim3(rows + 1), dim3(64), 0, s, table, rows, proj_b, nw, K, eps, (u32x4*)xtab, stab);
+}
+
 #define BG_PH(RT_, NT_) ((8 * (RT_) * (NT_) > 64 && ((RT_) * (NT_)) % 2 == 0) ? 2 : 1)
-template <int RT, int NT, int D, bool NTW, bool Q8>
+template <int RT, int NT, int D, bool NTW, bool Q8, bool FOLD = false>
 __global__ __launch_bounds__(512) void k_bgemm(Q3BGemm g) {
     extern __shared__ float part[];
     __shared__ float srow[64];
@@ -52,7 +175,13 @@
     for (int j = 0; j < NT; ++j) wp[j] = (const u32x4*)g.w + ((size_t)(nb0 + j) * kblocks + kb0) * 64 + lane;
     constexpr int NR = 2 * RT;
     float sp0[NR], sp1[NR];
-    if (g.ssp) {
+    [[maybe_unused]] BgFold<RT> fs;
+    [[maybe_unused]] int* scode = (int*)part;
+    if constexpr (FOLD) {
+        fs.phase1(g, row0, cg, wave, lane);
+        __builtin_amdgcn_sched_barrier(0);
+    }
+    if (!FOLD && g.ssp) {
 #pragma unroll
         for (int i = 0; i < NR; ++i) {
             const float* sp = g.ssp + (size_t)min(row0 + wave + 8 * i, B - 1) * g.ld_ssp;
@@ -90,11 +219,13 @@
 #pragma unroll
             for (int j = 0; j < NT; ++j) bq[s][j] = bg_ldw(wp[j] + so, NTW);
         }
-#pragma unroll
-        for (int s = 0; s < D; ++s) {
-            const size_t so = (size_t)min(s, per - 1) * 64;
-#pragma unroll
-            for (int i = 0; i < RT; ++i) aq[s][i] = ap[i][so];
+        if constexpr (!FOLD) {
+#pragma unroll
+            for (int s = 0; s < D; ++s) {
+                const size_t so = (size_t)min(s, per - 1) * 64;
+#pragma unroll
+                for (int i = 0; i < RT; ++i) aq[s][i] = ap[i][so];
+            }
         }
     }
     constexpr int NOUT = (TR * 64 + 511) / 512;
@@ -124,7 +255,11 @@
     }
     __builtin_amdgcn_sched_barrier(0);
     Q3_STAMP(g, 1);
-    if (g.ssp) {
+    if constexpr (FOLD) {
+        fs.template phase2<D>(g, row0, wave, lane, kq, r, per, kb0, scode, aq);
+        Q3_STAMP(g, 7);
+    }
+    if (!FOLD && g.ssp) {
         float av[NR];
 #pragma unroll
         for (int i = 0; i < NR; ++i) {
@@ -209,7 +344,7 @@
 #ifdef Q3_STAMPS
                 if (s == 0) { asm volatile("" :: "v"(acc[0][0][0])); Q3_STAMP(g, 2); }
 #endif
-                if (s + D < per) {
+                if (!FOLD && s + D < per) {
 #pragma unroll
                     for (int j = 0; j < NT; ++j) bq[d][j] = bg_ldw(wp[j] + (size_t)(s + D) * 64, NTW);
 #pragma unroll
@@ -225,6 +360,11 @@
     constexpr int PH = BG_PH(RT, NT), TP = RT * NT / PH, TRP = TR / PH, NOUTP = NOUT / PH;
     static_assert(PH == 1 || ((RT * NT) % 2 == 0 && (TRP * 64) % 512 == 0), "two phases need an even tile count and whole items per phase");
     const int epi = g.epi;
+    const bool nrm = FOLD || g.ssp;
+    if constexpr (FOLD) {
+        fs.phase3(g, row0, cg, wave, lane, scode, srow);
+        Q3_LDS_BARRIER();
+    }
 #pragma unroll
     for (int ph = 0; ph < PH; ++ph) {
         if (ph) __syncthreads();
@@ -247,7 +387,7 @@
                 const int q = p & 31, l = ((q >> 3) << 4) + (q & 7), o = ((p >> 5) << 6) + l;
                 const int e = (o >> 6) & 3, t = ph * TP + (o >> 8), i = t / NT, j = t - i * NT;
                 const int rl = 16 * i + 4 * (l >> 4) + e, row = row0 + rl, c = l & 15;
-                const float sc = g.ssp ? srow[rl] : 1.0f;
+                const float sc = nrm ? srow[rl] : 1.0f;
                 float gt = part[o], up = part[o + 8];
 #pragma unroll
                 for (int wv = 1; wv < 8; ++wv) { gt = gt + part[(size_t)wv * (TRP * 64) + o]; up = up + part[(size_t)wv * (TRP * 64) + o + 8]; }
@@ -263,13 +403,13 @@
             const int rl = 16 * i + 4 * (l >> 4) + e, row = row0 + rl, c = l & 15;
             const int col = (nb0 + j) * 16 + c;
             const bool live = row < B;
-            const float sc = g.ssp ? srow[rl] : 1.0f;
+            const float sc = nrm ? srow[rl] : 1.0f;
             float v = part[o];
 #pragma unroll
             for (int wv = 1; wv < 8; ++wv) v = v + part[(size_t)wv * (TRP * 64) + o];
             if (g.bias) v = v + bsv[it];
             if (epi == Q3_EPI_STORE) {
-                if (live) g.y[bg_yoff(g, row) + col] = g.ssp ? sc * v : v;
+                if (live) g.y[bg_yoff(g, row) + col] = nrm ? sc * v : v;
             } else if (epi == Q3_EPI_GELU) {
                 if (live) g.yb[q3_atile_off(row, col, g.N >> 5)] = q3_bf16(bg_gelu_erf(v));
             } else if (epi == Q3_EPI_RESID) {
@@ -283,7 +423,7 @@
                     if (live && c == 0) g.ssp_out[(size_t)row * g.ld_ssp_out + (nb0 + j)] = sq;
                 }
             } else {
-                unsigned long long key = q3_argmax_key(g.ssp ? sc * v : v, (uint32_t)col);
+                unsigned long long key = q3_argmax_key(nrm ? sc * v : v, (uint32_t)col);
 #pragma unroll
                 for (int m = 1; m <= 8; m <<= 1) { const unsigned long long ok = __shfl_xor(key, m); key = ok > key ? ok : key; }
                 if (live && c == 0) g.keys[(size_t)row * g.key_stride + (nb0 + j)] = key;
@@ -465,6 +605,13 @@
         } else if (nt) hipLaunchKernelGGL((k_bgemm<RT, NT, D, true, false>), grid, dim3(512), lds, s, g);
         else hipLaunchKernelGGL((k_bgemm<RT, NT, D, false, false>), grid, dim3(512), lds, s, g);
     }
+    static void launch_fold(const Q3BGemm& g, dim3 grid, hipStream_t s) {
+        if constexpr (NT == 1) {
+            const size_t fl = std::max(lds, (size_t)4 * RT * 16);
+            constexpr int DF = D < 4 ? D : 4;
+            hipLaunchKernelGGL((k_bgemm<RT, 1, DF, false, false, true>), grid, dim3(512), fl, s, g);
+        }
+    }
 };
 #define BG_EACH(X) X(1, 1) X(1, 2) X(1, 3) X(2, 1) X(2, 2) X(2, 3) X(3, 1) X(3, 2) X(3, 3) X(4, 1) X(4, 2) X(4, 3)
 static int g_lds_cap_kb = 0;
@@ -490,7 +637,7 @@
 
 static void bg_pick(const Q3BGemm& g, int* rt, int* nt, int* big) {
     *big = 0;
-    if (g.B >= 256 && g_force_rt == 0 && bg_big_ok(g)) {
+    if (g.B >= 256 && g_force_rt == 0 && !g.fold.keys && bg_big_ok(g)) {
         const int policy = g_big_policy;
         const long wgs = (long)(g.N / 128) * ((g.B + 127) / 128);
         if (policy > 0 || (policy == 0 && wgs >= 256)) { *big = 1; *rt = 8; *nt = 8; return; }
@@ -500,6 +647,7 @@
     for (int RT = 1; RT <= 4; ++RT)
         for (int NT = 1; NT <= 3; ++NT) {
             if (tiles % NT) continue;
+            if (g.fold.keys && NT != 1) continue;
             if (g_lds_cap_kb > 0 && 8 * RT * NT / BG_PH(RT, NT) > g_lds_cap_kb && !(RT == 1 && NT == 1)) continue;
             if (g.B > 64 && RT != 4 && !(RT == 2 && g.B <= 128)) continue;
             const long chunks = (g.B + 16 * RT - 1) / (16 * RT);
@@ -508,7 +656,7 @@
             const long cost = rounds * ((g.wscale ? 32L * RT + 17L * NT : 32L * (RT + NT)) * g.K + 24000L);
             if (bestCost < 0 || cost < bestCost || (cost == bestCost && (wgs > bestWgs || (wgs == bestWgs && NT > bestNT)))) { bestCost = cost; bestRT = RT; bestNT = NT; bestWgs = wgs; }
         }
-    if (g_force_rt > 0 && g_force_nt > 0 && tiles % g_force_nt == 0) { bestRT = g_force_rt; bestNT = g_force_nt; }
+    if (g_force_rt > 0 && g_force_nt > 0 && tiles % g_force_nt == 0 && !(g.fold.keys && g_force_nt != 1)) { bestRT = g_force_rt; bestNT = g_force_nt; }
     *rt = bestRT; *nt = bestNT;
 }
 void q3_bgemm_pick(const Q3BGemm& g, int* rt, int* nt, int* d, int* ntw, int* big) {
@@ -532,11 +680,26 @@
     return 0;
 }
 
+bool q3_bgemm_fold_ok(int B, int K, int N, int n_key_parts) {
+    return B >= 1 && K % 256 == 0 && K <= 1024 && N % 16 == 0 && n_key_parts >= 1 && n_key_parts <= 128;
+}
+
 int q3_launch_bgemm(const Q3BGemm& g, hipStream_t s) {
     if (bg_check(g)) return -1;
     q3_bgemm_prepare();
+    if (g.fold.keys && (!q3_bgemm_fold_ok(g.B, g.K, g.N, g.fold.n_key_parts) || g.epi != Q3_EPI_STORE || g.wscale || g.a_row0 || g.ssp ||
+                        g.ntiles != g.K / 16 || g.fold.d < 1 || g.bias || g.seg_rows))
+        return -1;
     int bestRT, bestNT, big;
     bg_pick(g, &bestRT, &bestNT, &big);
+    if (g.fold.keys) {
+        if (big || bestNT != 1) return -1;
+        const dim3 grid(g.N / 16, (g.B + 16 * bestRT - 1) / (16 * bestRT));
+#define L(RT_, NT_) if (bestRT == RT_ && bestNT == NT_) { BgInst<RT_, NT_>::launch_fold(g, grid, s); return 0; }
+        BG_EACH(L)
+#undef L
+        return -1;
+    }
     if (big) { bg_launch_big(g, s); return 0; }
     const dim3 grid(g.N / 16 / bestNT, (g.B + 16 * bestRT - 1) / (16 * bestRT));
 #define L(RT_, NT_) if (bestRT == RT_ && bestNT == NT_) { BgInst<RT_, NT_>::launch(g, grid, s); return 0; }
diff --git a/qwen3-tts-rust_amd/csrc/q3_engine.h b/qwen3-tts-rust_amd/csrc/q3_engine.h
--- a/qwen3-tts-rust_amd/csrc/q3_engine.h
+++ b/qwen3-tts-rust_amd/csrc/q3_engine.h
@@ -58,6 +58,7 @@
     std::vector<float*> codec;
     const float** codec_dev = nullptr;
     std::vector<float*> pproj;
+    std::vector<uint4*> fold_x; std::vector<float*> fold_s;
     float* proj_w = nullptr;
     float* proj_b = nullptr;
     float* tts_pad = nullptr;
@@ -87,6 +88,7 @@
     Q3Voc* voc = nullptr;
     Q3Mel* mel = nullptr;
     Q3Clone* clone = nullptr;
+    int pred_fold = 1;
     int probe = 0, probe_kind = 0;
     std::vector<hipEvent_t> probe_ev;
     int probe_i = 0;
diff --git a/qwen3-tts-rust_amd/csrc/q3_engine.hip b/qwen3-tts-rust_amd/csrc/q3_engine.hip
--- a/qwen3-tts-rust_amd/csrc/q3_engine.hip
+++ b/qwen3-tts-rust_amd/csrc/q3_engine.hip
@@ -288,7 +288,8 @@
 
 static int run_layers(q3tts_engine* e, Q3Tfm& t, float* x, uint16_t* xb, float* ssp, int rows, const int* row_pos, const int* row_slot, Q3Scratch& sc,
                        hipStream_t s, bool one_row_per_slot = false, hipEvent_t* probe = nullptr, int slot_mod = 0, int pos_const = 0,
-                       const int* seg = nullptr, int n_seg = 0, int seg_max_n = 0, uint16_t* xscale = nullptr, int x_rt16 = 0) {
+                       const int* seg = nullptr, int n_seg = 0, int seg_max_n = 0, uint16_t* xscale = nullptr, int x_rt16 = 0,
+                       const Q3BGemm::Fold* fold = nullptr) {
     auto gemm = [&](Q3BGemm& g) { return t.a8 ? q3_launch_bgemm8(g, s) : q3_launch_bgemm(g, s); };
     const float eps = e->cfg.model.rms_eps;
     int bad = 0;
@@ -300,6 +301,7 @@
         g.a = xb; g.B = rows; g.w = t.wqkv[l]; g.wscale = t.q8 ? t.sqkv[l] : nullptr; g.K = t.d; g.N = t.nqkv; g.ssp = ssp; g.ld_ssp = nt; g.ntiles = nt; g.d_norm = t.d; g.eps = eps;
         g.epi = Q3_EPI_STORE; g.y = sc.qkv; g.ldy = t.nqkv;
         if (t.a8) { g.ascale = xscale; g.a_rt16 = x_rt16; }
+        if (fold && l == 0) { g.fold = *fold; g.ssp = nullptr; }
         const int pk = (probe && l == 0) ? e->probe_kind : -1;
         if (pk == 1) hipEventRecord(probe[0], s);
         bad += gemm(g) != 0;
@@ -369,12 +371,19 @@
         if (last && e->T.a8) { pn.xscale = L.ascT; pn.x_rt16 = L.rt16T; }
         q3_launch_pred_next(pn, s);
     };
+    const bool fold = e->fold_x.size() == (size_t)ncb && e->fold_x[1] && q3_bgemm_fold_ok(B, dp, e->P.nqkv, cbs / 16);
     for (int q = 0; q < ncb - 1; ++q) {
         const int rows = q == 0 ? 2 * B : B;
-        if (q > 0) pred_next(q);
+        Q3BGemm::Fold fd{};
+        if (q > 0 && fold) {
+            fd.keys = L.keys; fd.n_key_parts = cbs / 16; fd.q = q; fd.ncb = ncb;
+            fd.xtab = e->fold_x[q]; fd.stab = e->fold_s[q]; fd.table = e->pproj[q]; fd.proj_b = e->proj_b; fd.codec = e->codec[q]; fd.rows_q = m.codecq_rows; fd.d = de;
+            fd.slots = slots; fd.row_slot = L.slot_id; fd.codes = codes; fd.max_steps_cap = cap; fd.fb = L.fb; fd.px = L.px;
+        } else if (q > 0) pred_next(q);
         hipEvent_t* pe = nullptr;
         if (e->probe == 1 && q == 1 && B == L.nb && e->probe_i + 2 <= 8) { pe = &e->probe_ev[e->probe_i]; e->probe_i += 2; }
-        bad += run_layers(e, e->P, L.px, L.xbP, L.sspP, rows, nullptr, nullptr, L.sc, s, q > 0, pe, B, q == 0 ? 0 : q + 1);
+        bad += run_layers(e, e->P, L.px, L.xbP, L.sspP, rows, nullptr, nullptr, L.sc, s, q > 0, pe, B, q == 0 ? 0 : q + 1,
+                          nullptr, 0, 0, nullptr, 0, fd.keys ? &fd : nullptr);
         Q3BGemm g{}; g.a = L.xbP; g.a_row0 = q == 0 ? B : 0; g.B = B; g.w = e->P.head + head_tile_stride * q; g.K = dp; g.N = cbs;
         g.ssp = q == 0 ? L.sspP + (size_t)B * (dp / 16) : L.sspP; g.ld_ssp = dp / 16; g.ntiles = dp / 16; g.d_norm = dp; g.eps = eps;
         g.epi = Q3_EPI_ARGMAX; g.keys = L.keys; g.key_stride = cbs / 16;
@@ -480,6 +489,7 @@
 #define HIPC(call) do { hipError_t er__ = (call); if (er__ != hipSuccess) { q3_set_err(e, Q3TTS_ERR_DEVICE, std::string(#call) + ": " + hipGetErrorString(er__)); return fail(Q3TTS_ERR_DEVICE); } } while (0)
     HIPC(hipSetDevice(cfg->device));
     q3_bgemm_prepare();
+    if (const char* ev = getenv("Q3TTS_PRED_FOLD")) e->pred_fold = atoi(ev) ? 1 : 0;
     HIPC(hipStreamCreateWithFlags(&e->stream, hipStreamNonBlocking));
     if (getenv("Q3TTS_VOC_SERIAL") && atoi(getenv("Q3TTS_VOC_SERIAL"))) e->vstream = e->stream;
     else if (getenv("Q3TTS_VOC_CUMASK")) {
@@ -536,6 +546,13 @@
         pj.y = e->pproj[q]; pj.ldy = m.p_d_model;
         q3_launch_project(pj, s);
     }
+    e->fold_x.assign(m.n_codebooks, nullptr); e->fold_s.assign(m.n_codebooks, nullptr);
+    if (e->pred_fold && !e->P.q8 && !e->P.a8 && q3_bgemm_fold_ok(1, m.p_d_model, e->P.nqkv, m.codebook_size / 16))
+        for (int q = 1; q < m.n_codebooks - 1; ++q) {
+            TRYC(dalloc(e, &e->fold_x[q], (size_t)(m.codecq_rows + 1) * m.p_d_model / 8));
+            TRYC(dalloc(e, &e->fold_s[q], (size_t)(m.codecq_rows + 1)));
+            q3_launch_fold_table(e->pproj[q], m.codecq_rows, e->proj_b, e->P.attn_norm[0], m.p_d_model, m.rms_eps, e->fold_x[q], e->fold_s[q], s);
+        }
     HIPC(hipStreamSynchronize(s));
     TRYC(dalloc(e, &e->slots, (size_t)B));
     HIPC(hipHostMalloc((void**)&e->slots_host, sizeof(Q3Slot) * 2 * B, hipHostMallocDefault));
@@ -641,7 +658,7 @@
         if (L.stream) hipStreamDestroy(L.stream);
     }
     free_tfm(e->T); free_tfm(e->P);
-    hipFree(e->text); for (auto p : e->codec) hipFree(p); for (auto p : e->pproj) hipFree(p); hipFree((void*)e->codec_dev); hipFree(e->proj_w); hipFree(e->proj_b);
+    hipFree(e->text); for (auto p : e->codec) hipFree(p); for (auto p : e->pproj) hipFree(p); for (auto p : e->fold_x) hipFree(p); for (auto p : e->fold_s) hipFree(p); hipFree((void*)e->codec_dev); hipFree(e->proj_w); hipFree(e->proj_b);
     hipFree(e->tts_pad_own); hipFree(e->marker_row); hipFree(e->dev_pcm);
     hipFree(e->slots); if (e->slots_host) hipHostFree(e->slots_host);
     hipFree(e->codes); hipFree(e->rng);
diff --git a/qwen3-tts-rust_amd/csrc/q3_kernels.h b/qwen3-tts-rust_amd/csrc/q3_kernels.h
--- a/qwen3-tts-rust_amd/csrc/q3_kernels.h
+++ b/qwen3-tts-rust_amd/csrc/q3_kernels.h
@@ -60,9 +60,19 @@
     unsigned long long* keys; int key_stride;
     const uint16_t* wscale;
     const uint16_t* ascale; int a_rt16; uint16_t* yscale; int y_rt16;
+    struct Fold {
+        const unsigned long long* keys; int n_key_parts; int q; int ncb;
+        const uint4* xtab; const float* stab;
+        const float* table; const float* proj_b;
+        const float* codec; int rows_q; int d;
+        const Q3Slot* slots; const int* row_slot; int* codes; int max_steps_cap;
+        float* fb; float* px;
+    } fold;
     Q3_STAMP_FIELD
 };
 int q3_launch_bgemm(const Q3BGemm& g, hipStream_t s);
+bool q3_bgemm_fold_ok(int B, int K, int N, int n_key_parts);
+void q3_launch_fold_table(const float* table, int rows, const float* proj_b, const float* nw, int K, float eps, uint4* xtab, float* stab, hipStream_t s);
 int q3_launch_bgemm8(const Q3BGemm& g, hipStream_t s);
 void q3_bgemm8_pick(const Q3BGemm& g, int* rt, int* nt);
 void q3_bgemm_pick(const Q3BGemm& g, int* rt, int* nt, int* d, int* ntw, int* big);
diff --git a/qwen3-tts-rust_amd/csrc/q3_kernels.hip b/qwen3-tts-rust_amd/csrc/q3_kernels.hip
--- a/qwen3-tts-rust_amd/csrc/q3_kernels.hip
+++ b/qwen3-tts-rust_amd/csrc/q3_kernels.hip
@@ -1211,6 +1211,7 @@
 }
 
 __global__ __launch_bounds__(256) void k_pred_next(Q3PredNext a) {
+    Q3_STAMP(a, 0);
     const int b = blockIdx.x, tid = threadIdx.x, d = a.d;
     unsigned long long kk = tid < a.n_key_parts ? a.keys[(size_t)b * a.n_key_parts + tid] : 0ull;
     const int slot = a.row_slot[b];
@@ -1286,6 +1287,10 @@
         __syncthreads();
         if (tid == 0) { a.row_pos_t[b] = sl->cur_pos; sl->cur_pos = sl->cur_pos + 1; sl->n_frames = frame + 1; }
     }
+#ifdef Q3_STAMPS
+    asm volatile("s_waitcnt vmcnt(0)" ::: "memory");
+    Q3_STAMP(a, 6);
+#endif
 }
 void q3_launch_pred_next(const Q3PredNext& a, hipStream_t s) { hipLaunchKernelGGL(k_pred_next, dim3(a.B), dim3(256), 0, s, a); }
 
```
